# llGuy/madrona_renderer

Hardware: AMD Instinct MI355X
Metric: rendered views/sec (whole node), N worlds x 64x64 RGB+depth (higher is better)
Workload: dtype f32

## Files before the change

include/mrx.h:

```cpp
#ifndef MRX_H
#define MRX_H

#include <stddef.h>
#include <stdint.h>

#ifdef __cplusplus
extern "C" {
#endif

#define MRX_ABI_VERSION 4

enum {
    MRX_OK = 0,
    MRX_E_INVALID = -1,
    MRX_E_NO_DEVICE = -2,
    MRX_E_HIP = -3,
    MRX_E_ASSET = -4,
    MRX_E_UNSUPPORTED = -5
};

enum { MRX_MODE_RASTERIZER = 0, MRX_MODE_RAYTRACER = 1 };

typedef struct {
    float position[3];
// ... 89 lines not shown
    uint32_t max_instances_per_world;
    const mrx_projection *camera_projections;
    const mrx_light *world_lights;
    const uint8_t *instance_colors;
    uint64_t reserved0;
} mrx_config;
#define MRX_CONFIG_V2_SIZE ((uint32_t)offsetof(mrx_config, device_ids))
#define MRX_CONFIG_V4_SIZE ((uint32_t)offsetof(mrx_config, camera_projections))
#define MRX_CONFIG_V4_PROJ_SIZE ((uint32_t)offsetof(mrx_config, world_lights))
#define MRX_CONFIG_V4_LIGHT_SIZE ((uint32_t)offsetof(mrx_config, instance_colors))

typedef struct mrx_renderer mrx_renderer;

enum {
    MRX_BUF_RGB = 0,
    MRX_BUF_DEPTH = 1,
    MRX_BUF_SEGMASK = 2,
    MRX_BUF_INSTANCE_POSITION = 3,
    MRX_BUF_INSTANCE_ROTATION = 4,
    MRX_BUF_CAMERA_POSITION = 5,
    MRX_BUF_CAMERA_ROTATION = 6,
    MRX_BUF_VISIBILITY = 7,
    MRX_BUF_INSTANCE_SCALE = 8,
    MRX_BUF_INSTANCE_OBJECT = 9,
    MRX_BUF_INSTANCE_COLOR = 10,
    MRX_NUM_BUFFERS = 11,
    MRX_BUF_INSTANCE_MATERIAL = 11,
    MRX_NUM_BUFFERS_EXT = 12,
    MRX_BUF_NORMAL = 12,
    MRX_NUM_BUFFERS_EXT2 = 13,
    MRX_BUF_INSTANCE_LABEL = 13,
    MRX_NUM_BUFFERS_EXT3 = 14
};

enum { MRX_DTYPE_U8 = 0, MRX_DTYPE_I32 = 1, MRX_DTYPE_F32 = 2 };

typedef struct {
    uint32_t num_worlds, num_views, num_instances;
    uint32_t num_objects, num_triangles, num_materials, num_textures;
    uint32_t max_world_triangles;
    uint32_t storage_fast, storage_slow;
    int32_t device_id;
    int32_t kernel_variant;
    uint64_t bytes_per_step;
    int32_t render_path;
    uint32_t bvh_nodes;
    uint32_t bvh_depth;
    uint32_t max_world_instances;
    uint32_t num_shards;
} mrx_info_t;
#define MRX_INFO_V2_SIZE ((size_t)offsetof(mrx_info_t, num_shards))

int mrx_create(const mrx_config *cfg, mrx_renderer **out);
void mrx_destroy(mrx_renderer *r);

int mrx_step(mrx_renderer *r);
int mrx_render(mrx_renderer *r);
int mrx_sync(mrx_renderer *r);

void *mrx_buffer(mrx_renderer *r, int which, int64_t dims[4], int *ndim,
                 int *dtype, int *device);

int mrx_supersample(mrx_renderer *r);
void *mrx_sample_buffer(mrx_renderer *r, int which, int64_t dims[4], int *ndim,
                        int *dtype, int *device);
int mrx_resolve(mrx_renderer *r);

int mrx_copy_to_host(mrx_renderer *r, int which, void *dst, uint64_t bytes);

int mrx_refresh_objects(mrx_renderer *r);

int mrx_num_shards(mrx_renderer *r);
mrx_renderer *mrx_shard(mrx_renderer *r, int shard);
void *mrx_buffer_shard(mrx_renderer *r, int shard, int which, int64_t dims[4], int *ndim,
                       int *dtype, int *device);
int64_t mrx_shard_first_world(mrx_renderer *r, int shard);
int64_t mrx_shard_split(uint32_t num_worlds, uint32_t shard, uint32_t num_shards);

enum {
    MRX_ENTRY_NONE = 0, MRX_ENTRY_GROUP_FAST = 1, MRX_ENTRY_GROUP = 2, MRX_ENTRY_CHUNKED = 3,
    MRX_ENTRY_BRUTE = 4, MRX_ENTRY_BVH = 5
};
int mrx_raster_entry(mrx_renderer *r);
enum { MRX_BVH_KERNEL_NONE = 0, MRX_BVH_KERNEL_TILE = 1, MRX_BVH_KERNEL_FLAT = 2 };
typedef struct {
    int32_t kernel;
    uint32_t tile_w, tile_h;
    uint32_t classify;
    uint32_t textured;
    uint32_t record_cap;
    uint32_t record_usable;
    uint32_t tex_cap;
    uint32_t big_cap;
    uint32_t pass_inst;
    uint32_t group_views;
    uint32_t mixed;
    uint32_t priority;
    uint32_t group_tiles;
    int32_t small_area;
    uint32_t workgroups;
} mrx_bvh_launch_t;
int mrx_bvh_launch(mrx_renderer *r, mrx_bvh_launch_t *out);
int mrx_info(mrx_renderer *r, mrx_info_t *out);
int mrx_info_sized(mrx_renderer *r, void *out, size_t size);
void *mrx_stream(mrx_renderer *r);
int mrx_set_stream(mrx_renderer *r, void *stream);

int mrx_time_renders(mrx_renderer *r, int steps, float *ms_total);
int mrx_time_steps_host(mrx_renderer *r, int steps, double *us_per_step);
int64_t mrx_debug_stamps(mrx_renderer *r, uint64_t *dst, int64_t capacity);
int mrx_mark(mrx_renderer *r, int which);
int mrx_elapsed_ms(mrx_renderer *r, float *ms);
int mrx_placement(mrx_renderer *r, float *cand_us, int capacity, float *kept_us);

int mrx_copy_triangles(mrx_renderer *r, float *tri_pos ,
                       float *tri_uv , int32_t *tri_mat ,
                       int32_t *obj_first , int32_t *obj_count );

int mrx_load_obj(const char *path, float **tri_pos, float **tri_uv,
                 uint32_t *num_tris);
int mrx_obj_objects(const char *path, uint32_t *first_tri, uint32_t capacity);
int mrx_decode_png(const char *path, uint8_t **rgba, uint32_t *width,
                   uint32_t *height);
int mrx_decode_texture(const char *path, uint8_t **rgba, uint32_t *width,
                       uint32_t *height);
int mrx_decode_bc7(const uint8_t *blocks, uint32_t num_blocks, uint8_t *rgba );
int64_t mrx_describe_obj_materials(const char *path, char *json, uint64_t capacity);
int mrx_blas_check(const float *tri_pos , uint32_t num_tris, uint32_t *num_nodes,
                   uint32_t *depth, uint32_t *num_leaves);
void mrx_free(void *p);
uint32_t mrx_dispatch_min_tris(uint32_t base, uint32_t num_views, int textured, uint32_t width, uint32_t height,
                               uint32_t num_cus);
uint32_t mrx_group_fill(uint32_t num_cus);
int mrx_dispatch_flat(int raytracer, uint32_t num_views, uint32_t width, uint32_t height, uint32_t max_world_triangles,
                      uint32_t max_world_instances, uint32_t num_cus);

int mrx_set_view_projection(mrx_renderer *r, uint32_t first_view, uint32_t count, const mrx_projection *proj);
int mrx_view_projection(mrx_renderer *r, uint32_t first_view, uint32_t count, mrx_projection *out);
int mrx_projection_constants(uint32_t width, uint32_t height, int render_mode, mrx_projection proj, float out[6]);

int mrx_set_world_light(mrx_renderer *r, uint32_t first_world, uint32_t count, const mrx_light *lights);
int mrx_world_light(mrx_renderer *r, uint32_t first_world, uint32_t count, mrx_light *out);
int mrx_light_constants(mrx_light light, float out[5]);

int mrx_set_instance_materials(mrx_renderer *r, uint32_t first_row, uint32_t count, const int32_t *materials);
int mrx_instance_materials(mrx_renderer *r, uint32_t first_row, uint32_t count, int32_t *out);

int mrx_set_instance_labels(mrx_renderer *r, uint32_t first_row, uint32_t count, const int32_t *labels);
int mrx_instance_labels(mrx_renderer *r, uint32_t first_row, uint32_t count, int32_t *out);

int mrx_device_count(void);
int mrx_abi_version(void);
const char *mrx_last_error(void);

#ifdef __cplusplus
}
#endif
#endif
```

madrona_renderer_amd/build.py:

```python
import os
import shutil
import subprocess
import sys
import sysconfig

HERE = os.path.dirname(os.path.abspath(__file__))
ROOT = os.path.dirname(HERE)
CSRC = os.path.join(HERE, "csrc")
ARCH = "gfx950"

HIP_SOURCES = ["raster.hip", "bvh.hip", "resolve.hip", "bvh.cpp", "mrx_api.cpp", "assets.cpp", "ktx2.cpp"]
HIP_DEPS = HIP_SOURCES + ["raster.hpp", "raster_dev.hpp", "bvh.hpp", "resolve.hpp", "assets.hpp", "bc7_tables.inc",
                          "../../include/mrx.h"]
MGR_SOURCES = ["manager.cpp"]
MGR_DEPS = MGR_SOURCES + ["../../include/madrona_mi355/manager.hpp",
                          "../../include/madrona_mi355/types.hpp", "../../include/mrx.h"]
PY_SOURCES = ["py_module.cpp", "manager.cpp"]


def ext_suffix():
    return sysconfig.get_config_var("EXT_SUFFIX") or ".so"


def lib_path():
    return os.path.join(HERE, "libmrx_hip.so")


def mgr_path():
    return os.path.join(HERE, "libmadrona_mi355.so")


def module_path():
    return os.path.join(HERE, "madrona_renderer" + ext_suffix())


def _stale(target, deps):
    if not os.path.exists(target):
        return True
    t = os.path.getmtime(target)
    return any(os.path.getmtime(os.path.join(CSRC, d)) > t for d in deps)


def _run(cmd, verbose):
    if verbose:
        print("+", " ".join(cmd), flush=True)
    subprocess.check_call(cmd)


def hipcc():
    exe = shutil.which("hipcc") or "/opt/rocm/bin/hipcc"
    if not os.path.exists(exe):
        raise RuntimeError("hipcc not found: the HIP library cannot be built")
    return exe


def build_hip(force=False, verbose=False, extra_flags=()):
    out = lib_path()
    if force or _stale(out, HIP_DEPS):
        cmd = [hipcc(), "--offload-arch=" + ARCH, "-O3", "-std=c++17", "-fPIC",
               "-shared", "-ffp-contract=off", "-fno-fast-math",
               "-mllvm", "-disable-promote-alloca-to-vector",
               "-fno-slp-vectorize",
               "-mllvm", "-amdgpu-kernarg-preload-count=12",
               "-Wall", "-Wno-unused-function"]
        cmd += list(extra_flags)
        cmd += os.environ.get("MRX_EXTRA_HIPCC_FLAGS", "").split()
        cmd += [os.path.join(CSRC, s) for s in HIP_SOURCES]
        cmd += ["-lz", "-ldl", "-Wl,-rpath,/opt/rocm/lib", "-o", out]
        _run(cmd, verbose)
    return out


def build_manager(force=False, verbose=False):
    out = mgr_path()
    if force or _stale(out, MGR_DEPS) or \
            os.path.getmtime(out) < os.path.getmtime(lib_path()):
        cmd = ["g++", "-O2", "-std=c++17", "-fPIC", "-shared", "-Wall"]
        cmd += [os.path.join(CSRC, s) for s in MGR_SOURCES]
        cmd += ["-L" + HERE, "-lmrx_hip", "-Wl,-rpath,$ORIGIN", "-o", out]
        _run(cmd, verbose)
    return out


def build_module(force=False, verbose=False):
    import pybind11
    out = module_path()
    if force or _stale(out, PY_SOURCES + MGR_DEPS) or \
            os.path.getmtime(out) < os.path.getmtime(lib_path()):
        cmd = ["g++", "-O2", "-std=c++17", "-fPIC", "-shared", "-Wall",
               "-fvisibility=hidden",
               "-I" + pybind11.get_include(),
               "-I" + sysconfig.get_paths()["include"]]
        cmd += [os.path.join(CSRC, s) for s in PY_SOURCES]
        cmd += ["-L" + HERE, "-lmrx_hip", "-Wl,-rpath,$ORIGIN", "-o", out]
        _run(cmd, verbose)
# ... 53 lines not shown
```

madrona_renderer_amd/csrc/mrx_api.cpp:

```cpp
#include "../../include/mrx.h"

#include <cmath>
#include <cstdio>
#include <cstdlib>
#include <cstring>
#include <algorithm>
#include <array>
#include <atomic>
#include <chrono>
#include <climits>
#include <map>
#include <string>
#include <thread>
#include <utility>
#include <vector>

#include <linux/futex.h>
#include <sys/syscall.h>
#include <unistd.h>

#include <hip/hip_runtime_api.h>

#include "assets.hpp"
#include "bvh.hpp"
// ... 220 lines not shown
        }
        return e;
    }
    const size_t tb = (px * 4 + kOutPeriod - 1) / kOutPeriod * kOutPeriod;
    const size_t depthOff = wantRgb ? tb + depthPhase : 0;
    const size_t idsOff = wantDepth ? depthOff + tb + kOutPeriod - (depthOff % kOutPeriod) + idsPhase
                                    : wantRgb ? tb + idsPhase : 0;
    const size_t end = (wantIds ? idsOff : wantDepth ? depthOff : 0) + px * 4;
    const size_t normalOff = (end + kOutPeriod - 1) / kOutPeriod * kOutPeriod + normalPhase;
    const size_t total = wantNormal ? normalOff + px * 4 : end;
    const char *how = std::getenv("MRX_OUT_ALLOC");
    int dev = 0;
    (void)hipGetDevice(&dev);
    auto own = [&](auto &buf) {
        return (how && how[0] == 'v') ? buf.allocVmm(px, total - px * 4, dev) : buf.alloc(px, total - px * 4);
    };
    const hipError_t e = wantRgb ? own(rgb) : wantDepth ? own(depth) : own(ids);
    if (e != hipSuccess)
        return e;
    char *base = static_cast<char *>(wantRgb ? rgb.base : wantDepth ? depth.base : ids.base);
    if (wantRgb && wantDepth)
        depth.view(base + depthOff, px);
    if (wantIds && (wantRgb || wantDepth))
        ids.view(base + idsOff, px);
    if (wantNormal)
        normal.view(base + normalOff, px);
    return hipSuccess;
}

}

struct ShardWorker;
static void stopShardWorkers(mrx_renderer *r);

struct mrx_renderer {
    int device = 0;
    hipStream_t stream = nullptr;
    int32_t mode = MRX_MODE_RASTERIZER;
    uint32_t flags = 0;
    int32_t variant = 0;
    uint64_t stepCount = 0;
    mrx_info_t info {};
    mrx::RasterParams params {};
    std::vector<mrx::ObjTri> hostTris;
    std::vector<int32_t> objFirst, objCount;
    DevBuf<mrx::ObjTri> tris;
    DevBuf<mrx::TriMat> triMats;
    DevBuf<mrx::TexDesc> textures;
    DevBuf<uint32_t> texels;
    DevBuf<mrx::WorldTri> viewTris;
    DevBuf<uint32_t> viewTriCount;
    DevBuf<uint8_t> poseBlock, geomBlock;
    DevBuf<float> instPos, instRot, instScale, camPos, camRot;
    DevBuf<int32_t> instObj;
    DevBuf<uint32_t> instColor;
    DevBuf<int32_t> instMat;
    DevBuf<mrx::MatRec> matTable;
    bool anyMatTextured = false;
    int32_t *matStage = nullptr;
    hipEvent_t matEv = nullptr;
    bool matCopyPending = false;
    DevBuf<int32_t> instLabel;
    int32_t *labelStage = nullptr;
    hipEvent_t labelEv = nullptr;
    bool labelCopyPending = false;
    DevBuf<uint32_t> rgb;
    DevBuf<float> depth;
    DevBuf<int32_t> ids;
    DevBuf<uint32_t> normal;
    uint32_t ss = 1;
    DevBuf<uint32_t> outRgb;
    DevBuf<float> outDepth;
    DevBuf<int32_t> outIds;
    DevBuf<uint32_t> outNormal;
    DevBuf<unsigned long long> stamps;
    uint32_t *xccHost = nullptr, *xccDev = nullptr;
    int32_t xcdPhaseForced = -1;
    uint32_t launches = 0;
    DevBuf<mrx::BvhNode> bvhNodes;
    DevBuf<uint32_t> bvhLeafTris, worldInstStart, viewWorld, instKBase;
    DevBuf<mrx::ObjInfo> objInfo;
    bool useBvh = false;
    int32_t lastEntry = mrx::kEntryNone;
    std::vector<int32_t> boundObj;
    std::vector<uint32_t> worldInstStartHost, viewWorldHost, worldCams;
    std::vector<mrx::TriMat> triMatsHost;
    mrx::BlasSet blas;
    uint32_t bvhMinTris = mrx::kBvhMinTris;
    uint32_t bvhGroupTilesGeneral = 1;
    std::vector<mrx_renderer *> shards;
    std::vector<uint32_t> shardFirstWorld;
    std::vector<ShardWorker *> workers;
    std::vector<mrx_renderer *> ownShards;
    uint32_t workerSeq = 0;
    bool shardAsync = false;
    uint32_t rendersPosted = 0;
    mrx_renderer *parent = nullptr;
    hipEvent_t ev0 = nullptr, ev1 = nullptr;
    std::vector<float> placementUs;
    float placementKeptUs = 0.0f;
    std::vector<mrx_projection> proj;
    DevBuf<mrx::ViewProj> projDev;
    mrx::ViewProj *projStage = nullptr;
    hipEvent_t projEv = nullptr;
    bool projCopyPending = false;
    std::vector<mrx_light> lights;
    DevBuf<mrx::ViewLight> lightDev;
    mrx::ViewLight *lightStage = nullptr;

    hipError_t launch()
    {
        const hipError_t e = launchRender();
        return e == hipSuccess && ss > 1 ? launchResolve() : e;
    }

    hipError_t launchResolve()
    {
        mrx::ResolveParams q {};
        q.rgbIn = params.rgb;
        q.depthIn = reinterpret_cast<const uint32_t *>(params.depth);
        q.idsIn = reinterpret_cast<const uint32_t *>(params.ids);
        q.normalIn = params.normal;
        q.rgbOut = outRgb.ptr;
        q.depthOut = reinterpret_cast<uint32_t *>(outDepth.ptr);
        q.idsOut = reinterpret_cast<uint32_t *>(outIds.ptr);
        q.normalOut = outNormal.ptr;
        q.rows = params.numViews * info.storage_slow;
        q.nfast = info.storage_fast;
        q.numCUs = params.numCUs;
        return mrx::launchResolve(q, (int)ss, stream);
    }

    hipError_t launchRender()
    {
        if (xcdPhaseForced >= 0)
            params.xcdPhase = (uint32_t)xcdPhaseForced;
        else if (xccHost)
            params.xcdPhase = *(volatile uint32_t *)xccHost & 1u;
        ++launches;
        params.xccReport = (xccDev && (launches <= 4 || (launches & 31u) == 0)) ? xccDev : nullptr;
        if (useBvh) {
            lastEntry = mrx::kEntryBvh;
            return mrx::launchBvh(params, stream);
        }
        return mrx::launchRaster(params, info.max_world_triangles, variant, stream, &lastEntry);
    }

    ~mrx_renderer()
    {
        stopShardWorkers(this);
        for (mrx_renderer *sh : shards)
            delete sh;
        if (!shards.empty())
            return;
        (void)hipSetDevice(device);
        tris.release(); triMats.release(); textures.release(); texels.release();
        viewTris.release(); viewTriCount.release();
        instPos.release(); instRot.release(); instScale.release();
        camPos.release(); camRot.release(); instObj.release(); instColor.release(); instMat.release();
        instLabel.release();
        matTable.release();
        projDev.release();
        lightDev.release();
        if (projStage)
            (void)hipHostFree(projStage);
        if (lightStage)
            (void)hipHostFree(lightStage);
        if (projEv)
            (void)hipEventDestroy(projEv);
        if (matStage)
            (void)hipHostFree(matStage);
        if (matEv)
            (void)hipEventDestroy(matEv);
        if (labelStage)
            (void)hipHostFree(labelStage);
        if (labelEv)
            (void)hipEventDestroy(labelEv);
        poseBlock.release(); geomBlock.release();
        rgb.release(); depth.release(); ids.release(); normal.release(); stamps.release();
        outRgb.release(); outDepth.release(); outIds.release(); outNormal.release();
        if (xccHost) (void)hipHostFree(xccHost);
        bvhNodes.release(); bvhLeafTris.release(); worldInstStart.release();
        viewWorld.release(); instKBase.release(); objInfo.release();
        if (ev0) (void)hipEventDestroy(ev0);
        if (ev1) (void)hipEventDestroy(ev1);
    }
};


enum : int { kCmdNone = 0, kCmdRender, kCmdSync, kCmdTimed, kCmdResolve, kCmdExit };

struct ShardWorker {
    std::vector<mrx_renderer *> shards;
    std::thread th;
    alignas(64) std::atomic<uint32_t> posted { 0 };
    std::atomic<int> cmd { kCmdNone };
    std::atomic<int> steps { 0 };
    alignas(64) std::atomic<uint32_t> sleeping { 0 };
    alignas(64) std::atomic<uint32_t> done { 0 };
    int rc = MRX_OK;
    std::string err;
    int64_t tSeen = 0, tDone = 0;
    alignas(64) std::atomic<uint32_t> masterSleeping { 0 };
    bool async = false;
    alignas(64) std::atomic<uint32_t> renderPosted { 0 };
    alignas(64) std::atomic<uint32_t> renderDone { 0 };
};

namespace {

inline void cpuRelax() { __builtin_ia32_pause(); }

inline long futexWait(std::atomic<uint32_t> *word, uint32_t expected)
{
    return syscall(SYS_futex, reinterpret_cast<uint32_t *>(word), FUTEX_WAIT_PRIVATE, expected, nullptr, nullptr, 0);
}

inline long futexWake(std::atomic<uint32_t> *word)
{
    return syscall(SYS_futex, reinterpret_cast<uint32_t *>(word), FUTEX_WAKE_PRIVATE, INT_MAX, nullptr, nullptr, 0);
}

int64_t shardSpinNs()
{
    static const int64_t ns = [] {
        const char *e = std::getenv("MRX_SHARD_SPIN_US");
        return (int64_t)(e ? std::max(0, std::atoi(e)) : 200) * 1000;
    }();
    return ns;
}

bool shardTrace()
{
    static const bool on = std::getenv("MRX_SHARD_TRACE") != nullptr;
    return on;
}

struct ShardTrace { int64_t wake = 0, launch = 0, own = 0, total = 0, n = 0; };
thread_local ShardTrace g_trace;

int64_t nowNs()
{
    return std::chrono::duration_cast<std::chrono::nanoseconds>(
               std::chrono::steady_clock::now().time_since_epoch()).count();
}

int groupRun(const std::vector<mrx_renderer *> &shards, int cmd, int steps, bool bindDevice)
{
    if (shards.empty())
        return MRX_OK;
    if (bindDevice)
        MRX_HIP(hipSetDevice(shards[0]->device));
    switch (cmd) {
    case kCmdRender:
        for (mrx_renderer *sh : shards)
            MRX_HIP(sh->launch());
        return MRX_OK;
    case kCmdResolve:
        for (mrx_renderer *sh : shards)
            MRX_HIP(sh->launchResolve());
        return MRX_OK;
    case kCmdSync:
// ... 914 lines not shown
    p.instPos = r.instPos.ptr;
    p.instRot = r.instRot.ptr;
    p.instScale = r.instScale.ptr;
    p.instObj = r.instObj.ptr;
    p.instColor = (cfg.flags & MRX_FLAG_NO_RGB) ? nullptr : r.instColor.ptr;
    p.instMat = (cfg.flags & MRX_FLAG_NO_RGB) ? nullptr : r.instMat.ptr;
    p.matTable = r.matTable.ptr;
    p.numMaterials = wantMats ? (uint32_t)allMats.size() : 0u;
    p.instLabel = (cfg.flags & MRX_FLAG_VISIBILITY_IDS) ? nullptr : r.instLabel.ptr;
    p.camPos = r.camPos.ptr;
    p.camRot = r.camRot.ptr;
    p.rgb = r.rgb.ptr;
    p.depth = r.depth.ptr;
    p.ids = wantIds ? r.ids.ptr : nullptr;
    p.normal = r.normal.ptr;
    p.numViews = nviews;
    {
        int cus = 0;
        MRX_HIP(hipDeviceGetAttribute(&cus, hipDeviceAttributeMultiprocessorCount, r.device));
        p.numCUs = (uint32_t)std::max(cus, 1);
        if (const char *dbg = std::getenv("MRX_FAKE_CUS"))
            p.numCUs = (uint32_t)std::max(1, std::atoi(dbg));
    }
    p.nfast = nfast;
    p.nslow = nslow;
    p.tilesFast = (nfast + 63) / 64;
    p.tilesSlow = (nslow + 63) / 64;
    for (mrx_projection &q : r.proj) {
        mrx::ViewProj c;
        if (projectionConstants(W, H, rt, q, c, &q) != MRX_OK)
            return MRX_E_INVALID;
    }
    p.invFar = rt ? 1.0f / kRtZFar : 0.0f;
    {
        const int rc = applyViewTables(r);
        if (rc != MRX_OK)
            return rc;
    }
    p.transposed = rt ? 1 : 0;
    p.idsAreSegmask = ((rt || wantLabels) && !(cfg.flags & MRX_FLAG_VISIBILITY_IDS)) ? 1 : 0;
    p.debugSkip = 0;
    if (const char *dbg = std::getenv("MRX_DEBUG_SKIP"))
        p.debugSkip = (uint32_t)std::atoi(dbg);
    p.debugStamps = nullptr;
    if (const char *dbg = std::getenv("MRX_DEBUG_STAMPS"))
        if (std::atoi(dbg) != 0) {
            const size_t n = ((size_t)nviews * p.tilesFast * p.tilesSlow * 4 + 64) * 4 * 8;
            MRX_HIP(r.stamps.alloc(n));
            MRX_HIP(hipMemset(r.stamps.ptr, 0, n * sizeof(unsigned long long)));
            p.debugStamps = r.stamps.ptr;
        }
    p.writeThrough = 1;
    if (const char *dbg = std::getenv("MRX_WRITE_THROUGH"))
        p.writeThrough = std::atoi(dbg) != 0;
    p.grpViews = p.grpChunkTiles = p.grpPerView = 0;
    p.grpViewsWanted = p.grpTilesWanted = 0;
    if (const char *dbg = std::getenv("MRX_GROUP_VIEWS"))
        p.grpViewsWanted = std::atoi(dbg);
    if (const char *dbg = std::getenv("MRX_GROUP_TILES"))
        p.grpTilesWanted = std::atoi(dbg);
    p.xcdRotate = 0;
    p.xcdRotateWanted = -1;
    if (const char *dbg = std::getenv("MRX_XCD_ROTATE"))
        p.xcdRotateWanted = std::atoi(dbg);
    p.xccReport = nullptr;
    p.xcdPhase = 0;
    if (hipHostMalloc((void **)&r.xccHost, 64, hipHostMallocMapped) == hipSuccess &&
        hipHostGetDevicePointer((void **)&r.xccDev, r.xccHost, 0) == hipSuccess) {
        *r.xccHost = 0;
        p.xccReport = r.xccDev;
    } else {
        (void)hipGetLastError();
        r.xccHost = nullptr;
    }
    if (const char *dbg = std::getenv("MRX_XCD_PHASE"))
        r.xcdPhaseForced = std::atoi(dbg) & 1;
    p.xcdSkew = 0;
    p.xcdSkewWanted = -1;
    if (const char *dbg = std::getenv("MRX_XCD_SKEW"))
        p.xcdSkewWanted = std::atoi(dbg);
    p.debugSlots = 0;
    if (const char *dbg = std::getenv("MRX_DEBUG_SLOTS"))
        p.debugSlots = std::atoi(dbg);
    p.bvhNodes = r.bvhNodes.ptr;
    p.bvhLeafTris = r.bvhLeafTris.ptr;
    p.numObjects = (uint32_t)r.objFirst.size();
    p.bvhUniInst = p.bvhUniCams = 0;
    if (cfg.num_worlds > 0) {
        bool uni = true;
        const uint32_t rows0 = worldInstStart[1] - worldInstStart[0];
        for (uint32_t w = 1; uni && w < cfg.num_worlds; ++w)
            uni = worldInstStart[w + 1] - worldInstStart[w] == rows0 &&
                  cfg.worlds[w].num_cameras == cfg.worlds[0].num_cameras;
        if (uni && rows0 > 0 && cfg.worlds[0].num_cameras > 0) {
            p.bvhUniInst = rows0;
            p.bvhUniCams = cfg.worlds[0].num_cameras;
        }
    }
    p.worldInstStart = r.worldInstStart.ptr;
    p.viewWorld = r.viewWorld.ptr;
    p.bvhPassInst = std::min<uint32_t>(128u, std::max<uint32_t>(8u, (maxWorldInst + 7u) / 8u * 8u));
    p.bvhTile = 0;
    if (const char *dbg = std::getenv("MRX_BVH_TILE"))
        p.bvhTile = std::max(0, std::min(2, std::atoi(dbg)));
    p.bvhClassify = blas.nodes.empty() ? 0 : 1;
    if (const char *dbg = std::getenv("MRX_BVH_CLASSIFY"))
        p.bvhClassify = std::atoi(dbg) != 0;
    p.bvhSmallArea = 256;
    if (const char *dbg = std::getenv("MRX_BVH_SMALL_AREA"))
        p.bvhSmallArea = std::max(0, std::min(4096, std::atoi(dbg)));
    if (const char *dbg = std::getenv("MRX_BVH_PASS_INST"))
        p.bvhPassInst = std::min<uint32_t>(512u, std::max<uint32_t>(8u, (uint32_t)std::atoi(dbg) / 8u * 8u));
    p.bvhGroupTiles = 1;
    if (maxWorldInst <= p.bvhPassInst) {
        const uint32_t tw = p.bvhTile == 2 ? 32 : 64, thh = p.bvhTile == 0 ? 64 : 32;
        const uint32_t tpv = ((nfast + tw - 1) / tw) * ((nslow + thh - 1) / thh);
        uint32_t g = 1;
        while (g < 16u && g * 2u <= tpv && (uint64_t)nviews * ((tpv + 2u * g - 1) / (2u * g)) >= 2u * p.numCUs)
            g *= 2;
        p.bvhGroupTiles = std::max(1u, g);
        if (const char *dbg = std::getenv("MRX_BVH_GROUP_TILES"))
            p.bvhGroupTiles = (uint32_t)std::max(1, std::min((int)tpv, std::atoi(dbg)));
    }
    r.bvhGroupTilesGeneral = p.bvhGroupTiles;
    mrx_info_t &inf = r.info;
    inf.num_worlds = cfg.num_worlds;
    inf.num_views = nviews;
    inf.num_instances = (uint32_t)instObj.size();
    inf.num_objects = (uint32_t)r.objFirst.size();
    inf.num_triangles = (uint32_t)tris.size();
    inf.num_materials = (uint32_t)allMats.size();
    inf.num_textures = (uint32_t)texDescs.size();
    inf.storage_fast = nfast;
    inf.storage_slow = nslow;
    inf.device_id = r.device;
    inf.kernel_variant = r.variant;
    inf.bvh_nodes = (uint32_t)blas.nodes.size();
    inf.bvh_depth = blas.maxDepth;
    inf.max_world_instances = maxWorldInst;
    inf.num_shards = 1;
    inf.bytes_per_step = (uint64_t)px * (4u * ((r.rgb.ptr ? 1u : 0u) + (r.depth.ptr ? 1u : 0u) + (r.normal.ptr ? 1u : 0u)) +
                                         (wantIds ? 4u : 0u)) +
                         (44ull + (r.instColor.ptr ? 4ull : 0ull) + (r.instMat.ptr ? 4ull : 0ull) +
                          (r.instLabel.ptr ? 4ull : 0ull)) * inf.num_instances +
                         28ull * nviews;
    return bindGeometry(r);
}

}

extern "C" {

int mrx_abi_version(void) { return MRX_ABI_VERSION; }

const char *mrx_last_error(void) { return g_err.c_str(); }

static std::vector<std::pair<mrx_renderer *, uint32_t>> viewOwners(mrx_renderer *r)
{
    std::vector<std::pair<mrx_renderer *, uint32_t>> out;
    uint32_t base = 0;
    if (r->shards.empty()) {
        out.emplace_back(r, 0u);
        return out;
    }
    for (mrx_renderer *sh : r->shards) {
        out.emplace_back(sh, base);
// ... 592 lines not shown
    }
    top->shardFirstWorld.push_back(cfg->num_worlds);
    startShardWorkers(top);
    *out = top;
    return MRX_OK;
}

void mrx_destroy(mrx_renderer *r)
{
    if (!r)
        return;
    stopShardWorkers(r);
    for (mrx_renderer *sh : r->shards) {
        (void)hipSetDevice(sh->device);
        (void)hipStreamSynchronize(sh->stream);
    }
    if (r->shards.empty()) {
        (void)hipSetDevice(r->device);
        (void)hipStreamSynchronize(r->stream);
    }
    delete r;
}

int mrx_render(mrx_renderer *r)
{
    if (r && r->parent) {
        const int src = settle(r);
        if (src != MRX_OK)
            return src;
    }
    if (!r)
        return fail(MRX_E_INVALID, "null renderer");
    if (!r->shards.empty())
        return shardsRun(r, kCmdRender);
    MRX_HIP(hipSetDevice(r->device));
    MRX_HIP(r->launch());
    return MRX_OK;
}

int mrx_step(mrx_renderer *r)
{
    if (!r)
        return fail(MRX_E_INVALID, "null renderer");
    r->stepCount++;
    return mrx_render(r);
}

int mrx_sync(mrx_renderer *r)
{
    if (r && r->parent) {
        const int src = settle(r);
        if (src != MRX_OK)
            return src;
    }
    if (!r)
        return fail(MRX_E_INVALID, "null renderer");
    if (!r->shards.empty())
        return shardsRun(r, kCmdSync);
    MRX_HIP(hipSetDevice(r->device));
    MRX_HIP(hipStreamSynchronize(r->stream));
    return MRX_OK;
}

void *mrx_stream(mrx_renderer *r) { return r ? (void *)r->stream : nullptr; }

static int wantsShard(const char *what)
{
    return fail(MRX_E_UNSUPPORTED, std::string(what) + ": this renderer spans several devices -- "
                                   "address one shard (mrx_shard / mrx_buffer_shard)");
}

static_assert(mrx::kEntryNone == MRX_ENTRY_NONE && mrx::kEntryGroupFast == MRX_ENTRY_GROUP_FAST &&
                  mrx::kEntryGroup == MRX_ENTRY_GROUP && mrx::kEntryChunked == MRX_ENTRY_CHUNKED &&
                  mrx::kEntryBrute == MRX_ENTRY_BRUTE && mrx::kEntryBvh == MRX_ENTRY_BVH,
              "raster.hpp RasterEntry and mrx.h MRX_ENTRY_* disagree");

int mrx_raster_entry(mrx_renderer *r)
{
    if (!r)
        return fail(MRX_E_INVALID, "null renderer");
    return r->shards.empty() ? r->lastEntry : r->shards[0]->lastEntry;
}

int mrx_bvh_launch(mrx_renderer *r, mrx_bvh_launch_t *out)
{
    if (!r)
        return fail(MRX_E_INVALID, "null renderer");
    if (!out)
        return fail(MRX_E_INVALID, "null output");
    const mrx_renderer &sh = r->shards.empty() ? *r : *r->shards[0];
    const mrx::BvhLaunchShape s = mrx::bvhLaunchShape(sh.params);
    mrx_bvh_launch_t o = {};
    o.kernel = !sh.useBvh ? MRX_BVH_KERNEL_NONE : s.flat ? MRX_BVH_KERNEL_FLAT : MRX_BVH_KERNEL_TILE;
    o.tile_w = s.tileW;
    o.tile_h = s.tileH;
    o.classify = s.classify;
    o.textured = s.textured;
    o.record_cap = s.recordCap;
    o.record_usable = s.recordUsable;
    o.tex_cap = s.texCap;
    o.big_cap = s.bigCap;
    o.pass_inst = s.passInst;
    o.group_views = s.groupViews;
    o.mixed = s.mixed;
    o.priority = s.priority;
    o.group_tiles = s.groupTiles;
    o.small_area = s.smallArea;
    o.workgroups = s.workgroups;
    *out = o;
    return MRX_OK;
}

int mrx_num_shards(mrx_renderer *r) { return !r ? 0 : r->shards.empty() ? 1 : (int)r->shards.size(); }

mrx_renderer *mrx_shard(mrx_renderer *r, int shard)
{
    if (!r || shard < 0 || shard >= mrx_num_shards(r)) {
        fail(MRX_E_INVALID, "no such shard");
        return nullptr;
    }
    return r->shards.empty() ? r : r->shards[shard];
}

void *mrx_buffer_shard(mrx_renderer *r, int shard, int which, int64_t dims[4], int *ndim, int *dtype,
                       int *device)
{
    mrx_renderer *sh = mrx_shard(r, shard);
    return sh ? mrx_buffer(sh, which, dims, ndim, dtype, device) : nullptr;
}

int64_t mrx_shard_split(uint32_t num_worlds, uint32_t shard, uint32_t num_shards)
{
    if (num_shards == 0 || shard > num_shards)
        return fail(MRX_E_INVALID, "bad shard");
    return (int64_t)shardFirstWorld(num_worlds, shard, num_shards);
}

int64_t mrx_shard_first_world(mrx_renderer *r, int shard)
{
    if (!r || shard < 0 || shard > mrx_num_shards(r))
        return fail(MRX_E_INVALID, "no such shard");
    if (r->shards.empty())
        return shard == 0 ? 0 : (int64_t)r->info.num_worlds;
    return (int64_t)r->shardFirstWorld[shard];
}

int mrx_refresh_objects(mrx_renderer *r)
{
    {
        const int src = settle(r);
        if (src != MRX_OK)
            return src;
    }
    if (!r)
        return fail(MRX_E_INVALID, "null renderer");
    for (mrx_renderer *sh : r->shards) {
        const int rc = mrx_refresh_objects(sh);
        if (rc != MRX_OK)
            return rc;
    }
    if (!r->shards.empty())
        return MRX_OK;
    MRX_HIP(hipSetDevice(r->device));
    MRX_HIP(hipStreamSynchronize(r->stream));
    std::vector<int32_t> live(r->boundObj.size());
    if (!live.empty())
// ... 454 lines not shown
        return fail(MRX_E_ASSET, err);
    *width = img.width;
    *height = img.height;
    *rgba = (uint8_t *)std::malloc(img.rgba.size() + 4);
    std::memcpy(*rgba, img.rgba.data(), img.rgba.size());
    return MRX_OK;
}

int mrx_decode_texture(const char *path, uint8_t **rgba, uint32_t *width, uint32_t *height)
{
    if (!path || !rgba || !width || !height)
        return fail(MRX_E_INVALID, "null argument");
    mrx::Image img;
    std::string err;
    if (!mrx::decodeTexture(path, img, err))
        return fail(MRX_E_ASSET, err);
    *width = img.width;
    *height = img.height;
    *rgba = (uint8_t *)std::malloc(img.rgba.size() + 4);
    std::memcpy(*rgba, img.rgba.data(), img.rgba.size());
    return MRX_OK;
}

int mrx_decode_bc7(const uint8_t *blocks, uint32_t num_blocks, uint8_t *rgba)
{
    if ((!blocks || !rgba) && num_blocks)
        return fail(MRX_E_INVALID, "null argument");
    for (uint32_t b = 0; b < num_blocks; ++b)
        mrx::decodeBC7Block(blocks + 16 * (size_t)b, reinterpret_cast<uint8_t (*)[4]>(rgba + 64 * (size_t)b));
    return MRX_OK;
}

int64_t mrx_describe_obj_materials(const char *path, char *json, uint64_t capacity)
{
    if (!path || !json)
        return fail(MRX_E_INVALID, "null argument");
    mrx::TriSoup soup;
    std::string err;
    if (!mrx::loadOBJ(path, soup, err))
        return fail(MRX_E_ASSET, err);
    auto quote = [](const std::string &s) {
        std::string o = "\"";
        for (char c : s) {
            if (c == '"' || c == '\\') o += '\\';
            o += c;
        }
        return o + "\"";
    };
    std::string out = "{\"num_tris\":" + std::to_string(soup.numTris()) + ",\"tri_mtl\":[";
    for (size_t i = 0; i < soup.triMtl.size(); ++i)
        out += (i ? "," : "") + std::to_string(soup.triMtl[i]);
    out += "],\"names\":[";
    for (size_t i = 0; i < soup.mtlNames.size(); ++i)
        out += (i ? "," : "") + quote(soup.mtlNames[i]);
    out += "],\"libs\":[";
    for (size_t i = 0; i < soup.mtlLibs.size(); ++i)
        out += (i ? "," : "") + quote(soup.mtlLibs[i]);
    out += "],\"materials\":[";
    std::vector<mrx::MtlMaterial> lib;
    for (const std::string &ml : soup.mtlLibs) {
        std::string merr;
        (void)mrx::loadMTL(ml, lib, merr);
    }
    for (size_t i = 0; i < lib.size(); ++i) {
        char kd[96];
        std::snprintf(kd, sizeof kd, "[%.9g,%.9g,%.9g]", lib[i].kd[0], lib[i].kd[1], lib[i].kd[2]);
        out += std::string(i ? "," : "") + "{\"name\":" + quote(lib[i].name) + ",\"kd\":" + kd +
               ",\"map_kd\":" + quote(lib[i].mapKd) + "}";
    }
    out += "]}";
    if (out.size() + 1 > capacity)
        return fail(MRX_E_INVALID, "buffer too small");
    std::memcpy(json, out.c_str(), out.size() + 1);
    return (int64_t)out.size();
}

uint32_t mrx_dispatch_min_tris(uint32_t base, uint32_t num_views, int textured, uint32_t width, uint32_t height,
                               uint32_t num_cus)
{
    return mrx::bvhDispatchMinTris(base ? base : mrx::kBvhMinTris, num_views, textured != 0, width, height, num_cus);
}

uint32_t mrx_group_fill(uint32_t num_cus) { return mrx::groupFill(num_cus); }

int mrx_dispatch_flat(int raytracer, uint32_t num_views, uint32_t width, uint32_t height, uint32_t max_world_triangles,
                      uint32_t max_world_instances, uint32_t num_cus)
{
    return mrx::bvhDispatchFlat(raytracer != 0, num_views, width, raytracer ? width : height, max_world_triangles,
                                max_world_instances, num_cus) ? 1 : 0;
}

int mrx_blas_check(const float *tri_pos, uint32_t num_tris, uint32_t *num_nodes, uint32_t *depth,
                   uint32_t *num_leaves)
{
    if ((!tri_pos && num_tris) || !num_nodes || !depth || !num_leaves)
        return fail(MRX_E_INVALID, "null argument");
    using namespace mrx;
    std::vector<ObjTri> tris(num_tris);
    for (uint32_t t = 0; t < num_tris; ++t)
        std::memcpy(tris[t].p, tri_pos + 9 * (size_t)t, 36);
    BlasSet b;
    buildBlas(tris.data(), { 0 }, { (int32_t)num_tris }, b);
    *num_nodes = (uint32_t)b.nodes.size();
    *depth = b.maxDepth;
    *num_leaves = 0;
    const ObjInfo &o = b.objects[0];
    if (o.root < 0)
        return num_tris <= kBvhFlatMax && b.nodes.empty() ? MRX_OK
                                                          : fail(MRX_E_INVALID, "large object without a hierarchy");
    if (1 + 7 * b.maxDepth > kBvhStackCap)
        return fail(MRX_E_INVALID, "hierarchy too deep for the traversal stack");
    std::vector<uint32_t> seen(num_tris, 0);
    struct Item { uint32_t node; float lo[3], hi[3]; };
    std::vector<Item> todo;
    {
        Item root {};
        root.node = (uint32_t)o.root;
        std::memcpy(root.lo, o.bbMin, 12);
        std::memcpy(root.hi, o.bbMax, 12);
        todo.push_back(root);
    }
    while (!todo.empty()) {
        const Item it = todo.back();
        todo.pop_back();
        if (it.node >= b.nodes.size())
            return fail(MRX_E_INVALID, "child index out of range");
        const BvhNode &n = b.nodes[it.node];
        for (uint32_t c = 0; c < kBvhWidth; ++c) {
            const uint32_t ref = n.child[c];
            if (ref == kBvhEmpty)
                continue;
            for (int a = 0; a < 3; ++a)
                if (n.bmin[c][a] < it.lo[a] || n.bmax[c][a] > it.hi[a])
                    return fail(MRX_E_INVALID, "child box sticks out of its parent's");
            if (ref & kBvhLeafBit) {
                const uint32_t cnt = ((ref >> kBvhLeafStartBits) & 15u) + 1u;
                const uint32_t start = ref & ((1u << kBvhLeafStartBits) - 1u);
                if (cnt > kBvhLeafMax || start + cnt > b.leafTris.size())
                    return fail(MRX_E_INVALID, "bad leaf");
                ++*num_leaves;
                for (uint32_t i = 0; i < cnt; ++i) {
                    const uint32_t t = b.leafTris[start + i];
                    if (t >= num_tris || seen[t]++)
                        return fail(MRX_E_INVALID, "triangle missing from or repeated in the leaves");
                    for (int v = 0; v < 3; ++v)
                        for (int a = 0; a < 3; ++a) {
                            const float x = tris[t].p[3 * v + a];
                            if (x < n.bmin[c][a] || x > n.bmax[c][a])
                                return fail(MRX_E_INVALID, "triangle outside its leaf's box");
                        }
                }
            } else {
                Item ch {};
                ch.node = ref;
                std::memcpy(ch.lo, n.bmin[c], 12);
                std::memcpy(ch.hi, n.bmax[c], 12);
                todo.push_back(ch);
            }
        }
    }
    for (uint32_t t = 0; t < num_tris; ++t)
        if (seen[t] != 1)
            return fail(MRX_E_INVALID, "triangle missing from the leaves");
    return MRX_OK;
}

// ... 4 lines not shown
```

madrona_renderer_amd/csrc/py_module.cpp:

```cpp
#include <pybind11/numpy.h>
#include <pybind11/pybind11.h>
#include <pybind11/stl.h>

#include <array>
#include <cmath>
#include <cstdio>
#include <string>
#include <vector>

#include "../../include/madrona_mi355/manager.hpp"
#include "../../include/mrx.h"

namespace py = pybind11;

namespace madRender {
namespace detail { void setThrowOnError(bool v); }
}

namespace {

using namespace madRender;

namespace {
struct PyCamera {
// ... 437 lines not shown
        .def("depth_cuda_ptr", [](py::object self, py::object shard) { return self.cast<Manager &>().depthCudaPtr(shardOf(self, shard)); },
             py::arg("shard") = py::none())
        .def("segmask_cuda_ptr", [](py::object self, py::object shard) { return self.cast<Manager &>().segmaskCudaPtr(shardOf(self, shard)); },
             py::arg("shard") = py::none())
        .def("instance_scale_tensor",
             [](py::object self, py::object shard) {
                 return wrapTensor(self, self.cast<Manager &>().instanceScaleTensor(shardOf(self, shard)));
             },
             py::arg("shard") = py::none())
        .def("refresh_objects", &Manager::refreshObjects)
        .def_property_readonly("num_shards", &Manager::numShards)
        .def("shard_first_world", &Manager::shardFirstWorld, py::arg("shard"))
        .def("instance_position_tensor",
             [](py::object self, py::object shard) {
                 return wrapTensor(self, self.cast<Manager &>().instancePositionTensor(shardOf(self, shard)));
             },
             py::arg("shard") = py::none())
        .def("instance_object_tensor",
             [](py::object self, py::object shard) {
                 return wrapTensor(self, self.cast<Manager &>().instanceObjectTensor(shardOf(self, shard)));
             },
             py::arg("shard") = py::none())
        .def("instance_color_tensor",
             [](py::object self, py::object shard) {
                 return wrapTensor(self, self.cast<Manager &>().instanceColorTensor(shardOf(self, shard)));
             },
             py::arg("shard") = py::none())
        .def("instance_label_tensor",
             [](py::object self, py::object shard) {
                 return wrapTensor(self, self.cast<Manager &>().instanceLabelTensor(shardOf(self, shard)));
             },
             py::arg("shard") = py::none())
        .def("instance_material_tensor",
             [](py::object self, py::object shard) {
                 return wrapTensor(self, self.cast<Manager &>().instanceMaterialTensor(shardOf(self, shard)));
             },
             py::arg("shard") = py::none())
        .def("instance_rotation_tensor",
             [](py::object self, py::object shard) {
                 return wrapTensor(self, self.cast<Manager &>().instanceRotationTensor(shardOf(self, shard)));
             },
             py::arg("shard") = py::none())
        .def("camera_position_tensor",
             [](py::object self, py::object shard) {
                 return wrapTensor(self, self.cast<Manager &>().cameraPositionTensor(shardOf(self, shard)));
             },
             py::arg("shard") = py::none())
        .def("camera_rotation_tensor",
             [](py::object self, py::object shard) {
                 return wrapTensor(self, self.cast<Manager &>().cameraRotationTensor(shardOf(self, shard)));
             },
             py::arg("shard") = py::none())
        .def("time_renders", &Manager::timeRenders, py::arg("steps"))
        .def("time_steps_host", &Manager::timeStepsHost, py::arg("steps"))
        .def("mark", &Manager::mark, py::arg("which"))
        .def("elapsed_ms", &Manager::elapsedMs)
        .def("bytes_per_step", &Manager::bytesPerStep)
        .def("render_path", [](Manager &self) { return std::string(self.renderPath()); })
        .def("raster_entry", [](Manager &self) { return std::string(self.rasterEntry()); })
        .def("bvh_launch",
             [](Manager &self) {
                 mrx_bvh_launch_t s = {};
                 if (mrx_bvh_launch(static_cast<mrx_renderer *>(self.nativeHandle()), &s) != MRX_OK)
                     throw std::runtime_error(mrx_last_error());
                 static const char *const kernels[] = {"none", "tile", "flat"};
                 py::dict d;
                 d["kernel"] = kernels[s.kernel >= 0 && s.kernel <= 2 ? s.kernel : 0];
                 d["tile"] = py::make_tuple(s.tile_w, s.tile_h);
                 d["classify"] = s.classify != 0;
                 d["textured"] = s.textured != 0;
                 d["record_cap"] = s.record_cap;
                 d["record_usable"] = s.record_usable;
                 d["tex_cap"] = s.tex_cap;
                 d["big_cap"] = s.big_cap;
                 d["pass_inst"] = s.pass_inst;
                 d["group_views"] = s.group_views;
                 d["mixed"] = s.mixed != 0;
                 d["priority"] = s.priority;
                 d["group_tiles"] = s.group_tiles;
                 d["small_area"] = s.small_area;
                 d["workgroups"] = s.workgroups;
                 return d;
             })
        .def("placement",
             [](Manager &self) {
                 float us[16] = {}, kept = 0.f;
                 const int n = self.placement(us, 16, &kept);
                 py::list cands;
                 for (int i = 0; i < n && i < 16; ++i)
                     cands.append(us[i]);
                 py::dict d;
                 d["tries"] = n > 0 ? n : 1;
                 d["candidates_us"] = cands;
                 d["kept_us"] = n > 0 ? py::object(py::float_(kept)) : py::object(py::none());
                 return d;
             })
        .def("native_handle", [](Manager &self) { return (uint64_t)self.nativeHandle(); })
        .def("set_camera_projection",
             [](Manager &self, py::object vfov, py::object znear, int64_t first_view) {
                 const int64_t total = (int64_t)self.numViews();
                 if (first_view < 0 || first_view > total)
                     throw py::value_error("first_view out of range");
                 auto asVec = [](py::object o, bool &scalar) {
                     std::vector<float> v;
                     scalar = !py::isinstance<py::sequence>(o) && !py::hasattr(o, "__len__");
                     if (scalar)
                         v.push_back(o.cast<float>());
                     else
                         v = py::array_t<float, py::array::c_style | py::array::forcecast>(o).cast<std::vector<float>>();
                     return v;
                 };
                 bool fs = true, zs = true;
                 std::vector<float> fv = asVec(vfov, fs), zv;
                 if (znear.is_none())
                     zv.push_back(0.0f);
                 else {
                     zv = asVec(znear, zs);
                     for (float z : zv)
                         znearOf(z);
                 }
                 if (!fs && !zs && fv.size() != zv.size())
                     throw py::value_error("vfov and znear differ in length");
                 const int64_t n = !fs ? (int64_t)fv.size() : !zs ? (int64_t)zv.size() : total - first_view;
                 if (first_view + n > total)
                     throw py::value_error("more projections than views from first_view on");
                 std::vector<Manager::CameraProjection> proj((size_t)n);
                 for (int64_t i = 0; i < n; ++i) {
                     proj[(size_t)i].vfovDeg = fs ? fv[0] : fv[(size_t)i];
                     proj[(size_t)i].znear = zs ? zv[0] : zv[(size_t)i];
                     checkProjection(proj[(size_t)i]);
                 }
                 if (!self.setViewProjection((uint32_t)first_view, (uint32_t)n, proj.data()))
                     throw py::value_error(mrx_last_error());
             },
             py::arg("vfov"), py::arg("znear") = py::none(), py::arg("first_view") = 0)
        .def("set_world_light",
             [](Manager &self, py::object direction, py::object ambient, py::object diffuse, int64_t first_world) {
                 const int64_t total = (int64_t)self.numWorlds();
                 if (first_world < 0 || first_world > total)
                     throw py::value_error("first_world out of range");
                 const py::array_t<float, py::array::c_style | py::array::forcecast> dir(direction);
                 const bool one = dir.ndim() == 1;
                 if (!((one && dir.shape(0) == 3) || (dir.ndim() == 2 && dir.shape(1) == 3)))
                     throw py::value_error("direction must be one (x, y, z) or an array of shape [n, 3]");
                 auto asVec = [](py::object o, bool &scalar) {
                     std::vector<float> v;
                     scalar = !py::isinstance<py::sequence>(o) && !py::hasattr(o, "__len__");
                     if (scalar)
                         v.push_back(o.cast<float>());
                     else
                         v = py::array_t<float, py::array::c_style | py::array::forcecast>(o).cast<std::vector<float>>();
                     return v;
                 };
                 bool as = true, ds = true;
                 std::vector<float> av, dv;
                 if (!ambient.is_none())
                     av = asVec(ambient, as);
                 if (!diffuse.is_none())
                     dv = asVec(diffuse, ds);
                 int64_t n = one ? -1 : (int64_t)dir.shape(0);
                 for (const auto &sv : { std::make_pair(as, &av), std::make_pair(ds, &dv) })
                     if (!sv.first) {
                         if (n >= 0 && (int64_t)sv.second->size() != n)
                             throw py::value_error("direction, ambient and diffuse differ in length");
                         n = (int64_t)sv.second->size();
                     }
// ... 98 lines not shown
```

madrona_renderer_amd/csrc/raster.hip:

```cpp
#include <hip/hip_runtime.h>
#include <algorithm>
#include <cstdlib>

#include "raster.hpp"
#include "raster_dev.hpp"

namespace mrx {
namespace {

constexpr int kWavesPerBlock = 4;
constexpr int kBruteThreads = kWave * kWavesPerBlock;
constexpr int kChunkedThreads = kWave * kWavesPerBlock, kChunkedWavesPerSimd = 3;
constexpr int kChunk = 64;
constexpr int kHot = 16;
constexpr int kBandRows = 16;
constexpr int kBlocksPerBand = 16;

struct WaveLds {
    float hot[kChunk][kHot];
    float cold[kChunk][kCold];
};

struct TileCtx {
    uint32_t view, tileX0, tileY0;
    uint32_t triBegin, numTris;
    int lx, ly;
};

template <bool PV>
__device__ __forceinline__ bool tileSetup(const RasterParams &p, uint32_t item, int lane,
                                          TileCtx &t, ViewConst &vc, ViewLight &lt)
{
    const uint32_t tilesPerView = p.tilesFast * p.tilesSlow;
    if (item >= p.numViews * tilesPerView)
        return false;
    t.view = item / tilesPerView;
    const uint32_t tile = item % tilesPerView;
    t.tileX0 = (tile % p.tilesFast) * 64u;
    t.tileY0 = (tile / p.tilesFast) * 64u;
    const float4 q = *reinterpret_cast<const float4 *>(p.camRot + 4 * t.view);
    if (PV)
        lt = viewLightOf(p, true, __builtin_amdgcn_readfirstlane(t.view));
    quatToMat(q.x, q.y, q.z, q.w, vc.Rc);
#pragma unroll
    for (int r = 0; r < 3; ++r) {
        vc.c[r] = p.camPos[3 * t.view + r];
        if (PV)
            vc.lv[r] = dot3(vc.Rc[0][r], vc.Rc[1][r], vc.Rc[2][r], lt.toLight[0], lt.toLight[1], lt.toLight[2]);
        else
            vc.lv[r] = dot3(vc.Rc[0][r], vc.Rc[1][r], vc.Rc[2][r],
                            p.toLight[0], p.toLight[1], p.toLight[2]);
    }
#pragma unroll
    for (int r = 0; r < 3; ++r) {
#pragma unroll
        for (int cc = 0; cc < 3; ++cc)
            vc.Rc[r][cc] = __uint_as_float(
                __builtin_amdgcn_readfirstlane(__float_as_uint(vc.Rc[r][cc])));
        vc.c[r] = __uint_as_float(__builtin_amdgcn_readfirstlane(__float_as_uint(vc.c[r])));
        vc.lv[r] = __uint_as_float(__builtin_amdgcn_readfirstlane(__float_as_uint(vc.lv[r])));
    }
    t.triBegin = t.view * p.viewTriStride;
    t.numTris = p.viewTriCount[t.view];
    t.lx = lane & 7;
    t.ly = lane >> 3;
    return true;
}

struct GroupSetupArgs {
    const ObjTri *tris;
    const TriMat *triMats;
    const float *instPos, *instRot, *instScale;
    float sx, ox, sz, oz, s6bPad, ambient, diffuse;
    int32_t transposed;
};

template <bool LAB = false, typename NRMOUT = NoNormalOut>
__device__ __forceinline__ bool setupTriangleProj(const RasterParams &p, const ViewProj &pr, const ViewLight &lt,
                                                  const ViewConst &vc, WorldTri wt, int32_t kWorld, TriPlanes &out,
                                                  float *shade, float *cold, const NRMOUT nrm = NRMOUT())
{
    const GroupSetupArgs sa = { p.tris, p.triMats, p.instPos, p.instRot, p.instScale,
                                pr.sx, pr.ox, pr.sz, pr.oz, pr.s6bPad, lt.ambient, lt.diffuse, p.transposed };
    InstXform x;
    instanceTransform(sa, vc, wt.inst, x);
// ... 411 lines not shown
            dst[1] = make_float4(c.B0, c.B1, c.B2, c.Dy);
            dst[2] = make_float4(c.C0, c.C1, c.C2, c.Dc);
            dst[3] = make_float4(__uint_as_float(mask), 0.f, 0.f, 0.f);
        }
        __syncthreads();

        const uint32_t left = t.numTris - pass;
        const int subs = left >= (uint32_t)kPass ? kWavesPerBlock : (int)((left + kWave - 1) / kWave);
#pragma unroll
        for (int g = 0; g < 4; ++g) {
            const int strip = 2 * wave + (g >> 1), hf = g & 1;
            const uint32_t fy = t.tileY0 + strip * 8 + t.ly;
            const float py = (float)fy;
            const uint32_t fx0 = t.tileX0 + hf * 32 + 4 * t.lx;
            float px[kRegionBlocks];
#pragma unroll
            for (int b = 0; b < kRegionBlocks; ++b)
                px[b] = (float)(fx0 + b);
            for (int sub = 0; sub < subs; ++sub) {
                const uint32_t mask = __float_as_uint(lds.planes[sub * kWave + lane][12]);
                const uint64_t act = __ballot((mask >> (2 * strip + hf)) & 1u);
                if (!(p.debugSkip & 2u))
                    rasterRegion<true, 0>(lds.planes, act, sub * kWave, px, py, invNear, best[g], bid[g]);
            }
#pragma unroll
            for (int b = 0; b < kRegionBlocks; ++b) {
                if (bid[g][b] >= 0) {
                    resolvePixel<IDS>(p, lds.rec, bid[g][b], best[g][b], px[b], py,
                                      outRgba[g][b], outId[g][b]);
                    if (NRM)
                        outNrm[g][b] = nrmLds[bid[g][b]];
                }
                bid[g][b] = -1;
            }
        }
    }

#pragma unroll
    for (int g = 0; g < 4; ++g) {
        const int strip = 2 * wave + (g >> 1), hf = g & 1;
        const uint32_t fy = t.tileY0 + strip * 8 + t.ly;
        const uint32_t fx0 = t.tileX0 + hf * 32 + 4 * t.lx;
        if (NRM)
            outputRegion<IDS, true>(p, t, fx0, fy, invFar, best[g], outRgba[g], outId[g], outNrm[g]);
        else
            outputRegion<IDS>(p, t, fx0, fy, invFar, best[g], outRgba[g], outId[g]);
    }
}

template <bool IDS>
__global__ __launch_bounds__(kChunkedThreads, kChunkedWavesPerSimd)
void rasterChunkedKernel(const RasterParams p)
{
    chunkedKernelBody<IDS, false>(p);
}

template <KernelForm F, bool IDS>
__global__ __launch_bounds__(kChunkedThreads, kChunkedWavesPerSimd)
void rasterChunkedFormKernel(const RasterParams p)
{
    static_assert(F == KernelForm::PV || F == KernelForm::N || F == KernelForm::NPV, "the forms of this family");
    chunkedKernelBody<IDS, formFlags(F).pv, formFlags(F).nrm>(p);
}

constexpr int kGroupTilesMax = 16;
constexpr int kGroupSlotsMax = 256;
constexpr int groupTilesMax(int slots) { return slots <= 128 ? kGroupTilesMax : 8; }

template <int SLOTS, bool PV = false>
struct GroupLds {
    static constexpr int kRecs = SLOTS <= kChunk ? kChunk + 16 : SLOTS;
    static constexpr int kBackground = kRecs;
    float planes[kRecs][16];
    uint32_t live[kRecs];
    float shade[kRecs + 1][4];
    float cold[kRecs][kCold];
    uint32_t masks[groupTilesMax(SLOTS) * (SLOTS <= kChunk ? kChunk : SLOTS)];
    uint32_t tileInfo[kGroupTilesMax][4];
    float tileNear[PV ? kGroupTilesMax : 1];
    uint32_t nextItem;
    uint8_t itemOrder[kGroupTilesMax * 8];
    uint2 items[SLOTS == 16 ? kGroupTilesMax * 8 : 1];
    uint8_t itemPos[SLOTS == 16 ? kGroupTilesMax * 8 : 1];
};
constexpr uint32_t kTileValid = 4u;
constexpr uint32_t kItemValid = 1u << 8;
constexpr uint32_t kItemNearFree = 1u << 9;
constexpr uint32_t kItemAnyTex = 1u << 10;


template <bool IDS, bool FULL, bool TEX, int OUT, bool NRM = false, typename LDS>
__device__ __forceinline__ void storeRegion(const RasterParams &p, const LDS &L, bool doRgb, bool doDepth,
                                            uint32_t *rgbTile, float *depthTile, int32_t *idsTile,
                                            uint32_t pixOff, uint32_t fx0, uint32_t fy,
                                            bool anyTex, const float (&px)[kRegionBlocks], float py,
                                            const float (&best)[kRegionBlocks],
                                            const int32_t (&bid)[kRegionBlocks],
                                            const uint32_t *nrmTab = nullptr, uint32_t *nrmTile = nullptr)
{
    uint32_t nrm[kRegionBlocks];
    if (NRM) {
#pragma unroll
        for (int b = 0; b < kRegionBlocks; ++b)
            nrm[b] = *reinterpret_cast<const uint32_t *>(reinterpret_cast<const char *>(nrmTab) + (bid[b] >> 2));
    }
    uint32_t rgba[kRegionBlocks];
    int32_t id[kRegionBlocks];
    float dep[kRegionBlocks];
    const char *shadeBase = reinterpret_cast<const char *>(&L.shade[0][0]);
#pragma unroll
    for (int b = 0; b < kRegionBlocks; ++b) {
        const float *h = reinterpret_cast<const float *>(shadeBase + bid[b]);
        if (OUT != kOutDepth)
            rgba[b] = __float_as_uint(h[0]);
        if (IDS)
            id[b] = __float_as_int(p.idsAreSegmask ? h[2] : h[3]);
        if (OUT != kOutRGB)
            dep[b] = bid[b] != LDS::kBackground * 16 ? __builtin_amdgcn_rcpf(best[b]) : 0.0f;
    }
    if (TEX && OUT != kOutDepth && anyTex && (OUT != kOutByPointer || doRgb)) {
#pragma unroll
        for (int b = 0; b < kRegionBlocks; ++b) {
            const int32_t rec = bid[b] >> 4;
            const int32_t tex = __float_as_int(L.shade[rec][1]);
            if (tex >= 0)
                rgba[b] = shadeTextured(p, L.cold[rec], tex, px[b], py, 1.0f / best[b]);
        }
    }
    if (p.debugSkip & 1u)
        return;
    if (FULL) {
        if (doRgb)
            streamStore16(p.writeThrough, rgbTile + pixOff, rgba[0], rgba[1], rgba[2], rgba[3]);
        if (doDepth)
            streamStore16(p.writeThrough, depthTile + pixOff, __float_as_uint(dep[0]), __float_as_uint(dep[1]),
                          __float_as_uint(dep[2]), __float_as_uint(dep[3]));
        if (IDS)
            streamStore16(p.writeThrough, idsTile + pixOff, (uint32_t)id[0], (uint32_t)id[1], (uint32_t)id[2], (uint32_t)id[3]);
        if (NRM)
            streamStore16(p.writeThrough, nrmTile + pixOff, nrm[0], nrm[1], nrm[2], nrm[3]);
    } else if (fy < p.nslow) {
#pragma unroll
        for (int b = 0; b < kRegionBlocks; ++b) {
            if (fx0 + b < p.nfast) {
                if (doRgb)
                    streamStore4(p.writeThrough, rgbTile + pixOff + b, rgba[b]);
                if (doDepth)
                    streamStore4(p.writeThrough, depthTile + pixOff + b, __float_as_uint(dep[b]));
                if (IDS)
                    streamStore4(p.writeThrough, idsTile + pixOff + b, (uint32_t)id[b]);
                if (NRM)
                    streamStore4(p.writeThrough, nrmTile + pixOff + b, nrm[b]);
            }
        }
    }
}

template <bool IDS, bool FULL, bool NRM = false>
__device__ __forceinline__ void storeBackground(const RasterParams &p, bool doRgb, bool doDepth, uint32_t *rgbTile,
                                                float *depthTile, int32_t *idsTile,
                                                uint32_t pixOff, uint32_t fx0, uint32_t fy, uint32_t *nrmTile = nullptr)
{
    if (p.debugSkip & 1u)
        return;
    const uint32_t bg = 0xFF000000u;
    if (FULL) {
        if (doRgb)
            streamStore16(p.writeThrough, rgbTile + pixOff, bg, bg, bg, bg);
        if (doDepth)
            streamStore16(p.writeThrough, depthTile + pixOff, 0u, 0u, 0u, 0u);
        if (IDS)
            streamStore16(p.writeThrough, idsTile + pixOff, ~0u, ~0u, ~0u, ~0u);
        if (NRM)
            streamStore16(p.writeThrough, nrmTile + pixOff, kNormalBackground, kNormalBackground, kNormalBackground,
                          kNormalBackground);
    } else if (fy < p.nslow) {
#pragma unroll
        for (int b = 0; b < kRegionBlocks; ++b) {
            if (fx0 + b < p.nfast) {
                if (doRgb)
                    streamStore4(p.writeThrough, rgbTile + pixOff + b, bg);
                if (doDepth)
                    streamStore4(p.writeThrough, depthTile + pixOff + b, 0u);
                if (IDS)
                    streamStore4(p.writeThrough, idsTile + pixOff + b, ~0u);
                if (NRM)
                    streamStore4(p.writeThrough, nrmTile + pixOff + b, kNormalBackground);
            }
        }
    }
}

template <typename LDS>
__device__ __forceinline__ uint32_t classifyPair(const LDS &L, int j, int k, int wave, float invNear, float invFar,
                                                 bool &nearOk, bool &tex)
{
    nearOk = false;
    tex = false;
    const uint32_t info = L.tileInfo[j][3];
    const int rec = (int)(info >> 8) + k;
    if (!(info & kTileValid) || !L.live[rec])
        return 0u;
    const float4 *src = reinterpret_cast<const float4 *>(L.planes[rec]);
    const float4 a = src[0], b = src[1], cc = src[2], bb = src[3];
    TriPlanes c;
    c.A0 = a.x; c.A1 = a.y; c.A2 = a.z; c.Dx = a.w;
    c.B0 = b.x; c.B1 = b.y; c.B2 = b.z; c.Dy = b.w;
    c.C0 = cc.x; c.C1 = cc.y; c.C2 = cc.z; c.Dc = cc.w;
    c.bbX0 = bb.x; c.bbX1 = bb.y; c.bbY0 = bb.z; c.bbY1 = bb.w;
    const uint32_t tx0 = L.tileInfo[j][1], ty0 = L.tileInfo[j][2];
    uint32_t m;
    switch (wave & 3) {
    case 0: m = classifyStrips<0, 2>(c, tx0, ty0, invNear, invFar, nearOk); break;
    case 1: m = classifyStrips<2, 4>(c, tx0, ty0, invNear, invFar, nearOk); break;
    case 2: m = classifyStrips<4, 6>(c, tx0, ty0, invNear, invFar, nearOk); break;
    default: m = classifyStrips<6, 8>(c, tx0, ty0, invNear, invFar, nearOk); break;
    }
    tex = __float_as_int(L.shade[rec][1]) >= 0;
    return m;
}

constexpr int groupWaves(bool tex) { return tex ? 4 : 8; }

template <bool IDS, int SLOTS, bool TEX, int XMODE, bool FAST, int OUT, bool PV = false, bool LT = false, bool COL = false,
          bool MAT = false, bool NRM = false, bool LAB = false>
__device__ __forceinline__ void groupKernelBody(const char *hPose, const char *hGeom, uint32_t hViews, uint32_t hInstances,
                                                uint32_t hPool, uint32_t hShape, uint32_t hGroups, uint32_t hPrefix,
                                                uint32_t hFirst01, uint32_t hFirst23, const RasterParams p)
{
    __shared__ GroupLds<SLOTS, PV> lds;
    constexpr int kBackground = GroupLds<SLOTS, PV>::kBackground;
    __shared__ uint32_t nrmLds[NRM ? GroupLds<SLOTS, PV>::kRecs + 1 : 1];
    const int wave = __builtin_amdgcn_readfirstlane(threadIdx.x / kWave);
    const int lane = threadIdx.x % kWave;
    if (!FAST || wave >= 2)
        touchKernelArguments<(FAST ? 48 : 0) + sizeof(RasterParams)>();
    const uint32_t aNumViews = FAST ? hViews : p.numViews;
    const uint32_t aGrpViews = FAST ? (hShape & 255u) : p.grpViews;
    const uint32_t aXcdSkew = FAST ? ((hShape >> 8) & 15u) : p.xcdSkew;
    const uint32_t aXcdRotate = FAST ? ((hShape >> 12) & 1u) : p.xcdRotate;
    const uint32_t aGrpPerView = FAST ? 1u : p.grpPerView;
    const uint32_t aGrid = FAST ? hGroups : gridDim.x;
    const uint32_t aUniInstances = FAST ? ((hShape >> 13) & 7u) : p.uniInstances;
    const uint32_t aUniCams = FAST ? ((hShape >> 16) & 255u) : p.uniCamsPerWorld;
    const uint32_t dskip = FAST ? 0u : p.debugSkip;
    const PoseLayout lay = poseLayout(hViews, hInstances);
    const float *aCamRot = FAST ? reinterpret_cast<const float *>(hPose + lay.camRot) : p.camRot;
    const float *aCamPos = FAST ? reinterpret_cast<const float *>(hPose + lay.camPos) : p.camPos;
    const int32_t *aInstObj = FAST ? reinterpret_cast<const int32_t *>(hPose + lay.instObj) : p.instObj;
    constexpr bool BYPTR = NRM || LAB;
    const uint32_t *aInstColor = BYPTR ? p.instColor
                                 : FAST ? reinterpret_cast<const uint32_t *>(hPose + lay.total)
                                 : MAT ? reinterpret_cast<const uint32_t *>(p.poseBlock + poseColorOffset(p.numViews, p.numInstances))
                                       : p.instColor;
    const int32_t *aInstMat = BYPTR ? p.instMat
                              : FAST ? reinterpret_cast<const int32_t *>(hPose + lay.total + mrxAlign256(hInstances * 4u))
                                     : p.instMat;
    const uint32_t tilesPerView = FAST ? 1u : p.tilesFast * p.tilesSlow;
    constexpr bool readyItems = FAST && !TEX;
    uint32_t firstView, groupViews, firstTile, groupTiles;
    const uint32_t blk = ((BYPTR ? (p.xcdPhase & 1u) != 0u : (XMODE & 1) != 0) && SLOTS == 16 && aXcdSkew && (blockIdx.x ^ 1u) < aGrid)
                             ? blockIdx.x ^ 1u : blockIdx.x;
    if (((XMODE & 2) || (BYPTR && SLOTS == 16)) && blockIdx.x == 0 && threadIdx.x == (groupWaves(TEX) - 1) * kWave && p.xccReport)
        *p.xccReport = __builtin_amdgcn_s_getreg((3 << 11) | 20);
    uint32_t bid = blk;
    if (aXcdRotate && (bid | 7u) < aGrid)
        bid = (bid & ~7u) | ((bid + 2u * (bid >> 3)) & 7u);
    if (aGrpPerView == 1) {
        firstView = bid * aGrpViews;
        groupViews = aGrpViews;
        firstTile = 0;
        groupTiles = groupViews * tilesPerView;
    } else {
        firstView = bid / aGrpPerView;
        groupViews = 1;
        firstTile = (bid - firstView * aGrpPerView) * p.grpChunkTiles;
        groupTiles = min(p.grpChunkTiles, tilesPerView - firstTile);
    }
    uint32_t firstStrip = 0, numStrips = groupTiles * 8;
    if (SLOTS == 16 && aXcdSkew) {
        if (blk & 1u) {
            firstStrip = aXcdSkew;
            numStrips -= aXcdSkew;
        } else {
            groupViews += 1;
            groupTiles += 1;
            numStrips += aXcdSkew;
        }
    }
    const int groupRecs = (int)groupViews * SLOTS;
    const int numPairs = (int)groupTiles * SLOTS;
    const float invNear = p.invNear, invFar = p.invFar;
    if (dskip & 16u)
        return;
    unsigned long long *stamps = (!FAST && p.debugStamps && wave < 4)
        ? p.debugStamps + ((size_t)blockIdx.x * 4 + wave) * 8 : nullptr;
#define MRX_STAMP(i)                                                           \
    do {                                                                       \
        if (stamps && lane == 0)                                               \
            stamps[i] = __builtin_amdgcn_s_memrealtime();                      \
    } while (0)
    MRX_STAMP(0);
    if (!readyItems)
        for (int i = threadIdx.x; i < numPairs; i += groupWaves(TEX) * kWave)
            lds.masks[i] = 0u;

    if (wave == groupWaves(TEX) - 1 && lane < (int)groupTiles) {
        uint32_t vi = (uint32_t)lane, tile = firstTile;
        if (tilesPerView != 1) {
            vi = groupViews == 1 ? 0u : (uint32_t)lane / tilesPerView;
            tile = firstTile + (uint32_t)lane - vi * tilesPerView;
        }
        const uint32_t ty = tilesPerView != 1 ? tile / p.tilesFast : 0u;
        lds.tileInfo[lane][0] = firstView + vi;
        lds.tileInfo[lane][1] = (tile - ty * p.tilesFast) * 64u;
        lds.tileInfo[lane][2] = ty * 64u;
        lds.tileInfo[lane][3] = (firstView + vi < aNumViews ? kTileValid : 0u) | ((vi * SLOTS) << 8);
        if (PV)
            lds.tileNear[lane] = firstView + vi < aNumViews ? viewProjOf(p, true, firstView + vi).invNear : 0.0f;
    }
    if (wave == groupWaves(TEX) - 1) {
        uint32_t base = 0;
        for (uint32_t c0 = 0; c0 < groupTiles * 8u; c0 += kWave) {
            const uint32_t c = c0 + (uint32_t)lane;
            uint32_t strip = c / groupTiles, tile = c - strip * groupTiles;
            if (tilesPerView != 1) {
                tile = c >> 3;
                strip = c & 7u;
            }
            const uint32_t g = tile * 8u + strip;
            const bool ok = strip < 8u && g >= firstStrip && g < firstStrip + numStrips;
            const uint64_t m = __ballot(ok);
            const uint32_t pos = base + __builtin_popcountll(m & ((1ull << lane) - 1ull));
            if (readyItems) {
                if (strip < 8u)
                    lds.itemPos[g] = ok ? (uint8_t)pos : (uint8_t)0xFF;
            } else if (ok) {
                lds.itemOrder[pos] = (uint8_t)g;
            }
            base += (uint32_t)__builtin_popcountll(m);
        }
    }
    if (wave * kWave < groupRecs) {
        const int rec = wave * kWave + lane;
        const int vi = rec / SLOTS, k = rec % SLOTS;
        const bool recOk = rec < groupRecs;
        const bool viewOk = recOk && firstView + vi < aNumViews;
        const uint32_t view = viewOk ? firstView + vi : 0u;
        WorldTri wt;
        uint32_t numTris;
        if (aUniInstances) {
            const uint32_t kk = (uint32_t)k;
            const uint32_t pre1 = FAST ? (hPrefix & 255u) : p.uniPrefix[1], pre2 = FAST ? ((hPrefix >> 8) & 255u) : p.uniPrefix[2];
            const uint32_t pre3 = FAST ? ((hPrefix >> 16) & 255u) : p.uniPrefix[3], pre4 = FAST ? (hPrefix >> 24) : p.uniPrefix[4];
            const uint32_t ft0 = FAST ? (hFirst01 & 0xFFFFu) : p.uniFirstTri[0], ft1 = FAST ? (hFirst01 >> 16) : p.uniFirstTri[1];
            const uint32_t ft2 = FAST ? (hFirst23 & 0xFFFFu) : p.uniFirstTri[2], ft3 = FAST ? (hFirst23 >> 16) : p.uniFirstTri[3];
            const uint32_t li = (kk >= pre1 ? 1u : 0u) + (kk >= pre2 ? 1u : 0u) + (kk >= pre3 ? 1u : 0u);
            const uint32_t pre = li == 0 ? 0u : li == 1 ? pre1 : li == 2 ? pre2 : pre3;
            const uint32_t first = li == 0 ? ft0 : li == 1 ? ft1 : li == 2 ? ft2 : ft3;
            uint32_t world = view;
            if (aUniCams != 1)
                world = view / aUniCams;
            wt.inst = world * aUniInstances + li;
            wt.tri = first + (kk - pre);
            numTris = viewOk ? pre4 : 0u;
            if (kk >= pre4) {
                wt.inst = 0;
                wt.tri = 0;
            }
        } else {
            wt = p.viewTris[view * p.viewTriStride + ((uint32_t)k < p.viewTriStride ? (uint32_t)k : 0u)];
            numTris = viewOk ? p.viewTriCount[view] : 0u;
        }
        ViewConst vc;
        const ViewLight lt = viewLightOf(p, PV && LT, view);
        {
            const float4 q = *reinterpret_cast<const float4 *>(aCamRot + 4 * view);
            quatToMat(q.x, q.y, q.z, q.w, vc.Rc);
#pragma unroll
            for (int r = 0; r < 3; ++r) {
                vc.c[r] = aCamPos[3 * view + r];
                vc.lv[r] = dot3(vc.Rc[0][r], vc.Rc[1][r], vc.Rc[2][r],
                                lt.toLight[0], lt.toLight[1], lt.toLight[2]);
            }
        }
        TriPlanes c;
        c.A0 = c.B0 = c.C0 = c.A1 = c.B1 = c.C1 = 0.0f;
        c.A2 = c.B2 = c.C2 = c.Dx = c.Dy = c.Dc = 0.0f;
        c.bbX0 = c.bbX1 = c.bbY0 = c.bbY1 = 0.0f;
        bool valid = false;
        MRX_STAMP(1);
        if (recOk) {
            lds.shade[rec][1] = __int_as_float(-1);
            if ((uint32_t)k < numTris && !(dskip & 8u)) {
                const ViewProj pr = viewProjOf(p, PV, view);
                const GroupSetupArgs sa = {
                    FAST ? reinterpret_cast<const ObjTri *>(hGeom) : p.tris,
                    FAST ? reinterpret_cast<const TriMat *>(hGeom + geomMatsOffset(hPool)) : p.triMats,
                    FAST ? reinterpret_cast<const float *>(hPose + lay.instPos) : p.instPos,
                    FAST ? reinterpret_cast<const float *>(hPose + lay.instRot) : p.instRot,
                    FAST ? reinterpret_cast<const float *>(hPose + lay.instScale) : p.instScale,
                    pr.sx, pr.ox, pr.sz, pr.oz, pr.s6bPad, lt.ambient, lt.diffuse, p.transposed };
                InstXform x;
                instanceTransform(sa, vc, wt.inst, x);
                if (BYPTR) {
                    const MatOverride mo = { aInstMat ? aInstMat[wt.inst] : -1, p.numMaterials, p.matTable };
                    if constexpr (NRM)
                        valid = setupTriangleCore<true, true, true, true>(sa, vc.lv, x, wt.tri, aInstObj[wt.inst], k, c,
                                                                          lds.shade[rec], lds.cold[rec],
                                                                          aInstColor ? aInstColor[wt.inst] : 0u, mo,
                                                                          NormalOut { nrmLds + rec });
                    else
                        valid = setupTriangleCore<true, true, true, true>(sa, vc.lv, x, wt.tri, aInstObj[wt.inst], k, c,
                                                                          lds.shade[rec], lds.cold[rec],
                                                                          aInstColor ? aInstColor[wt.inst] : 0u, mo);
                    if (LAB)
                        applyLabel(lds.shade[rec], p.instLabel, wt.inst);
                } else {
                const MatOverride mo = { MAT ? aInstMat[wt.inst] : -1, p.numMaterials, p.matTable };
                valid = setupTriangleCore<true, OUT != kOutDepth, COL, MAT>(sa, vc.lv, x, wt.tri, aInstObj[wt.inst], k, c,
                                                                            lds.shade[rec], lds.cold[rec],
                                                                            COL ? aInstColor[wt.inst] : 0u, mo);
                }
            }
            MRX_STAMP(2);
            float4 *dst = reinterpret_cast<float4 *>(lds.planes[rec]);
            dst[0] = make_float4(c.A0, c.A1, c.A2, c.Dx);
            dst[1] = make_float4(c.B0, c.B1, c.B2, c.Dy);
            dst[2] = make_float4(c.C0, c.C1, c.C2, c.Dc);
            dst[3] = make_float4(c.bbX0, c.bbX1, c.bbY0, c.bbY1);
            lds.live[rec] = (valid && !(dskip & 4u)) ? 1u : 0u;
        }
        if (rec == 0) {
            lds.nextItem = 0;
            lds.shade[kBackground][0] = __uint_as_float(0xFF000000u);
            lds.shade[kBackground][1] = __int_as_float(-1);
            lds.shade[kBackground][2] = __int_as_float(-1);
            lds.shade[kBackground][3] = __int_as_float(-1);
            if (NRM)
                nrmLds[kBackground] = kNormalBackground;
        }
    }
    __syncthreads();
    MRX_STAMP(3);

    constexpr int kPairStride = (groupWaves(TEX) / 4) * kWave;
    for (int pair = (wave >> 2) * kWave + lane; pair - lane < numPairs; pair += kPairStride) {
        if (readyItems) {
            uint32_t m = 0;
            bool nearOk = false, tex = false;
            if (pair < numPairs)
                m = classifyPair(lds, pair / SLOTS, pair % SLOTS, wave, PV ? lds.tileNear[pair / SLOTS] : invNear, invFar,
                                 nearOk, tex);
            m >>= 4 * (wave & 3);
            const uint64_t l0 = __ballot(m & 1u), r0 = __ballot(m & 2u), l1 = __ballot(m & 4u), r1 = __ballot(m & 8u);
            const uint64_t near0 = __ballot((m & 3u) && !nearOk), near1 = __ballot((m & 12u) && !nearOk);
            const uint64_t tex0 = __ballot((m & 3u) && tex), tex1 = __ballot((m & 12u) && tex);
            if (lane % 16 == 0 && pair < numPairs) {
                const uint32_t j = (uint32_t)pair / 16u;
                const uint32_t valid = firstView + j < aNumViews ? kItemValid : 0u;
                const auto put = [&](uint32_t strip, uint64_t l, uint64_t r, uint64_t nearHit, uint64_t texHit) {
                    const uint32_t pos = lds.itemPos[j * 8u + strip];
                    if (pos == 0xFFu)
                        return;
                    const uint32_t desc = j | strip << 4 | valid |
                                          (((nearHit >> lane) & 0xFFFFu) == 0 ? kItemNearFree : 0u) |
                                          (((texHit >> lane) & 0xFFFFu) != 0 ? kItemAnyTex : 0u);
                    lds.items[pos] = make_uint2((uint32_t)((l >> lane) & 0xFFFFu) | (uint32_t)((r >> lane) & 0xFFFFu) << 16,
                                                desc);
                };
                put(2u * (wave & 3), l0, r0, near0, tex0);
                put(2u * (wave & 3) + 1u, l1, r1, near1, tex1);
            }
            continue;
        }
        if (pair >= numPairs)
            continue;
        bool nearOk, tex;
        uint32_t m = classifyPair(lds, pair / SLOTS, pair % SLOTS, wave, PV ? lds.tileNear[pair / SLOTS] : invNear,
                                  invFar, nearOk, tex);
        if (nearOk)
            m |= 1u << (16 + (wave & 3));
        if (m)
            atomicOr(&lds.masks[pair], m);
    }
    __syncthreads();
    MRX_STAMP(4);

    const int lx = lane & 7, ly = lane >> 3;
    const uint32_t laneOff = (uint32_t)ly * p.nfast + 4u * lx;
    int cachedTile = -1, recBase = 0;
    constexpr int SUBS = (SLOTS + kWave - 1) / kWave;
    constexpr int LANES = SLOTS < kWave ? SLOTS : kWave;
    uint32_t view = 0, tileX0 = 0, tileY0 = 0, mask[SUBS] = {};
    float pxTile[2][kRegionBlocks] = {};
    bool anyTex = false, nearFree = false, full = false;
    uint32_t *rgbTile = nullptr;
    float *depthTile = nullptr;
    int32_t *idsTile = nullptr;
    uint32_t *nrmTile = nullptr;
    const bool doRgb = storesRgb<OUT>(p.rgb), doDepth = storesDepth<OUT>(p.depth);
    uint32_t itemMasks = 0;
    float tileNear = invNear;
    if (readyItems) {
        full = (p.nfast & 3u) == 0 && 64u <= p.nfast && 64u <= p.nslow;
#pragma unroll
        for (int hf = 0; hf < 2; ++hf)
#pragma unroll
            for (int b = 0; b < kRegionBlocks; ++b)
                pxTile[hf][b] = (float)(hf * 32 + 4 * lx + b);
    }
    for (;;) {
        uint32_t item = 0;
        if (lane == 0)
            item = atomicAdd(&lds.nextItem, 1u);
        item = __builtin_amdgcn_readfirstlane(item);
        if (item >= numStrips)
            break;
        int j, strip;
        if (readyItems) {
            const uint2 d = lds.items[item];
            itemMasks = __builtin_amdgcn_readfirstlane(d.x);
            const uint32_t desc = __builtin_amdgcn_readfirstlane(d.y);
            if (!(desc & kItemValid))
                continue;
            j = (int)(desc & 15u);
            strip = (int)((desc >> 4) & 7u);
            nearFree = (desc & kItemNearFree) != 0;
            anyTex = (desc & kItemAnyTex) != 0;
            recBase = j * SLOTS;
            if (PV)
                tileNear = __uint_as_float(__builtin_amdgcn_readfirstlane(__float_as_uint(lds.tileNear[j])));
            const size_t tileBase = (size_t)(firstView + (uint32_t)j) * p.nslow * p.nfast;
            rgbTile = p.rgb + tileBase;
            depthTile = p.depth + tileBase;
            idsTile = IDS ? p.ids + tileBase : nullptr;
            nrmTile = NRM ? p.normal + tileBase : nullptr;
        } else {
            item = __builtin_amdgcn_readfirstlane((uint32_t)lds.itemOrder[item]);
            j = (int)(item >> 3);
            strip = (int)(item & 7u);
            if (j != cachedTile) {
                const uint32_t info = __builtin_amdgcn_readfirstlane(lds.tileInfo[j][3]);
                if (!(info & kTileValid))
                    continue;
                cachedTile = j;
                recBase = (int)(info >> 8);
                view = __builtin_amdgcn_readfirstlane(lds.tileInfo[j][0]);
                tileX0 = __builtin_amdgcn_readfirstlane(lds.tileInfo[j][1]);
                tileY0 = __builtin_amdgcn_readfirstlane(lds.tileInfo[j][2]);
                if (PV)
                    tileNear = __uint_as_float(__builtin_amdgcn_readfirstlane(__float_as_uint(lds.tileNear[j])));
                const size_t tileBase = ((size_t)view * p.nslow + tileY0) * p.nfast + tileX0;
                rgbTile = p.rgb + tileBase;
                depthTile = p.depth + tileBase;
                idsTile = IDS ? p.ids + tileBase : nullptr;
                nrmTile = NRM ? p.normal + tileBase : nullptr;
                full = (p.nfast & 3u) == 0 && tileX0 + 64u <= p.nfast && tileY0 + 64u <= p.nslow;
                anyTex = false;
                nearFree = true;
#pragma unroll
                for (int sub = 0; sub < SUBS; ++sub) {
                    const int slot = sub * kWave + lane;
                    mask[sub] = lane < LANES ? lds.masks[j * SLOTS + slot] : 0u;
                    const int32_t tex = lane < LANES ? __float_as_int(lds.shade[recBase + slot][1]) : -1;
                    anyTex = anyTex || __ballot((mask[sub] & 0xFFFFu) != 0 && tex >= 0) != 0;
                    nearFree = nearFree &&
                               __ballot((mask[sub] & 0xFFFFu) != 0 && ((mask[sub] >> 16) & 0xFu) != 0xFu) == 0;
                }
#pragma unroll
                for (int hf = 0; hf < 2; ++hf)
#pragma unroll
                    for (int b = 0; b < kRegionBlocks; ++b)
                        pxTile[hf][b] = (float)(tileX0 + hf * 32 + 4 * lx + b);
            }
        }
        const uint32_t fy = tileY0 + strip * 8 + ly;
        const float py = (float)fy;
#pragma unroll
        for (int hf = 0; hf < 2; ++hf) {
            const uint32_t fx0 = tileX0 + hf * 32 + 4 * lx;
            const uint32_t pixOff = (uint32_t)(strip * 8) * p.nfast + hf * 32 + laneOff;
            uint64_t act[SUBS];
            bool any = false;
#pragma unroll
            for (int sub = 0; sub < SUBS; ++sub) {
                act[sub] = readyItems ? (uint64_t)((itemMasks >> (16 * hf)) & 0xFFFFu)
                                     : __ballot((mask[sub] >> (2 * strip + hf)) & 1u);
                any = any || act[sub] != 0;
            }
            if (!any) {
                if (full)
                    storeBackground<IDS, true, NRM>(p, doRgb, doDepth, rgbTile, depthTile, idsTile, pixOff, fx0, fy, nrmTile);
                else
                    storeBackground<IDS, false, NRM>(p, doRgb, doDepth, rgbTile, depthTile, idsTile, pixOff, fx0, fy, nrmTile);
                continue;
            }
            const float (&px)[kRegionBlocks] = pxTile[hf];
            float best[kRegionBlocks];
            int32_t bid[kRegionBlocks];
#pragma unroll
            for (int b = 0; b < kRegionBlocks; ++b) {
                best[b] = invFar;
                bid[b] = kBackground * 16;
            }
            if (!(dskip & 2u)) {
#pragma unroll
                for (int sub = 0; sub < SUBS; ++sub) {
                    if (SUBS > 1 && act[sub] == 0)
                        continue;
                    if (nearFree)
                        rasterRegion<false, 4>(lds.planes, act[sub], recBase + sub * kWave, px, py, tileNear, best, bid);
                    else
                        rasterRegion<true, 4>(lds.planes, act[sub], recBase + sub * kWave, px, py, tileNear, best, bid);
                }
            }
            if (full)
                storeRegion<IDS, true, TEX, OUT, NRM>(p, lds, doRgb, doDepth, rgbTile, depthTile, idsTile, pixOff, fx0, fy,
                                                      anyTex, px, py, best, bid, nrmLds, nrmTile);
            else
                storeRegion<IDS, false, TEX, OUT, NRM>(p, lds, doRgb, doDepth, rgbTile, depthTile, idsTile, pixOff, fx0, fy,
                                                       anyTex, px, py, best, bid, nrmLds, nrmTile);
        }
    }
    MRX_STAMP(5);
    MRX_STAMP(6);
    if (stamps && lane == 0)
        stamps[7] = ((unsigned long long)__builtin_amdgcn_s_getreg((31 << 11) | 20) << 32) |
                    (unsigned long long)__builtin_amdgcn_s_getreg((31 << 11) | 4);
#undef MRX_STAMP
}

constexpr int groupThreads(bool tex) { return kWave * groupWaves(tex); }
constexpr int groupWavesPerSimd(KernelForm f, int slots, bool tex)
{
    if (tex)
        return slots > 128 ? 3 : 4;
    if (formFlags(f).lt)
        return 6;
    if (f == KernelForm::N)
        return slots >= 128 ? 6 : 8;
    return slots > 128 ? 6 : 8;
}

template <bool IDS, int SLOTS, bool TEX, int XMODE = 0, int OUT = kOutRGBD>
__global__ __launch_bounds__(groupThreads(TEX), groupWavesPerSimd(KernelForm::Uniform, SLOTS, TEX))
void rasterGroupKernel(const RasterParams p)
{
    groupKernelBody<IDS, SLOTS, TEX, XMODE, false, OUT>(nullptr, nullptr, 0u, 0u, 0u, 0u, 0u, 0u, 0u, 0u, p);
}

template <bool IDS, bool TEX, int XMODE, int OUT>
__global__ __launch_bounds__(groupThreads(TEX), groupWavesPerSimd(KernelForm::Uniform, 16, TEX))
void rasterGroupKernelFast(const char *hPose, const char *hGeom, uint32_t hViews, uint32_t hInstances, uint32_t hPool,
                           uint32_t hShape, uint32_t hGroups, uint32_t hPrefix, uint32_t hFirst01, uint32_t hFirst23,
                           const RasterParams p)
{
    groupKernelBody<IDS, 16, TEX, XMODE, true, OUT>(hPose, hGeom, hViews, hInstances, hPool, hShape, hGroups, hPrefix, hFirst01,
                                               hFirst23, p);
}

template <KernelForm F, bool IDS, int SLOTS, bool TEX>
__global__ __launch_bounds__(groupThreads(TEX), groupWavesPerSimd(F, SLOTS, TEX))
void rasterGroupFormKernel(const RasterParams p)
{
    constexpr FormFlags f = formFlags(F);
    static_assert(F != KernelForm::Uniform && F != KernelForm::PVM && (IDS || !f.lab), "the forms of this family");
    groupKernelBody<IDS, SLOTS, TEX, 0, false, kOutByPointer, f.pv, f.lt, f.col, f.mat, f.nrm, f.lab>(
        nullptr, nullptr, 0u, 0u, 0u, 0u, 0u, 0u, 0u, 0u, p);
}

template <KernelForm F, bool IDS, bool TEX>
__global__ __launch_bounds__(groupThreads(TEX), groupWavesPerSimd(F, 16, TEX))
void rasterGroupFormKernelFast(const char *hPose, const char *hGeom, uint32_t hViews, uint32_t hInstances, uint32_t hPool,
                               uint32_t hShape, uint32_t hGroups, uint32_t hPrefix, uint32_t hFirst01, uint32_t hFirst23,
                               const RasterParams p)
{
    constexpr FormFlags f = formFlags(F);
    static_assert(F != KernelForm::Uniform && F != KernelForm::PVM && (IDS || !f.lab), "the forms of this family");
    groupKernelBody<IDS, 16, TEX, 0, true, kOutByPointer, f.pv, f.lt, f.col, f.mat, f.nrm, f.lab>(
        hPose, hGeom, hViews, hInstances, hPool, hShape, hGroups, hPrefix, hFirst01, hFirst23, p);
}

KernelForm tileForm(const RasterParams &p)
{
    if (p.normal && p.viewProj) return KernelForm::NPV;
    if (p.normal)               return KernelForm::N;
    if (p.viewProj)             return KernelForm::PV;
    return KernelForm::Uniform;
}
KernelForm groupForm(const RasterParams &p)
{
    const bool pv = p.viewProj != nullptr;
    if (p.instLabel && p.ids && pv)       return p.normal ? KernelForm::LN : KernelForm::L;
    if (p.normal && pv && p.tablesVary)   return KernelForm::NPV;
    if (p.normal)                         return KernelForm::N;
    if (p.instMat && pv && p.tablesVary)  return KernelForm::PVLM;
    if (p.instMat)                        return KernelForm::M;
    if (p.instColor && pv && p.tablesVary) return KernelForm::PVLC;
    if (p.instColor)                      return KernelForm::C;
    if (pv && p.lightTable)               return KernelForm::PVL;
    if (pv)                               return KernelForm::PV;
    return KernelForm::Uniform;
}

}

hipError_t launchRaster(const RasterParams &p, uint32_t maxWorldTris,
                        int32_t variant, hipStream_t stream, int32_t *entry)
{
    const uint32_t items = p.numViews * p.tilesFast * p.tilesSlow;
    if (items == 0)
        return hipSuccess;
    const dim3 block(kWave * kWavesPerBlock);
    const bool ids = p.ids != nullptr;
    const bool multi = maxWorldTris > (uint32_t)kChunk;
    const bool large = maxWorldTris > (uint32_t)kGroupSlotsMax;
    if (variant == kVariantBrute) {
        if (entry) *entry = kEntryBrute;
        const dim3 grid((items + kWavesPerBlock - 1) / kWavesPerBlock);
        const KernelForm form = tileForm(p);
        const OutSel out = outSelOf(p.rgb, p.depth);
        const auto byIdsMulti = [&](auto f) {
            withBool(ids, [&](auto IDS) { withBool(multi, [&](auto MULTI) { f(IDS, MULTI); }); });
        };
        if (form != KernelForm::Uniform)
            withValue<KernelForm, KernelForm::NPV, KernelForm::N, KernelForm::PV>(form, [&](auto F) {
                byIdsMulti([&](auto IDS, auto MULTI) {
                    rasterBruteFormKernel<decltype(F)::value, decltype(IDS)::value, decltype(MULTI)::value><<<grid, block, 0, stream>>>(p);
                });
            });
        else
            withValue<int, kOutDepth, kOutRGB, kOutRGBD>(out, [&](auto O) {
                byIdsMulti([&](auto IDS, auto MULTI) {
                    rasterBruteKernel<decltype(IDS)::value, decltype(MULTI)::value, decltype(O)::value><<<grid, block, 0, stream>>>(p);
                });
            });
    } else if (large) {
        if (entry) *entry = kEntryChunked;
        const KernelForm form = tileForm(p);
        withBool(ids, [&](auto IDS) {
            constexpr bool kIds = decltype(IDS)::value;
            if (form != KernelForm::Uniform)
                withValue<KernelForm, KernelForm::PV, KernelForm::N, KernelForm::NPV>(form, [&](auto F) {
                    rasterChunkedFormKernel<decltype(F)::value, kIds><<<dim3(items), block, 0, stream>>>(p);
                });
            else
                rasterChunkedKernel<kIds><<<dim3(items), block, 0, stream>>>(p);
        });
    } else {
        int slots = 16;
        while ((uint32_t)slots < maxWorldTris)
            slots *= 2;
        if (p.debugSlots >= slots && p.debugSlots <= kGroupSlotsMax && (p.debugSlots & (p.debugSlots - 1)) == 0)
            slots = p.debugSlots;
        const uint32_t tpv = p.tilesFast * p.tilesSlow;
        const uint32_t maxTiles = (uint32_t)groupTilesMax(slots);
        const uint32_t kFill = groupFill(p.numCUs);
        RasterParams q = p;
        uint32_t vg = 1, ct = tpv, gpv = 1;
        if (tpv == 1) {
            vg = std::max<uint32_t>(1u, (uint32_t)(kChunk / slots));
            if (p.anyTextured)
                vg = std::min<uint32_t>(vg, 2u);
            while (vg > 1 && (p.numViews + vg - 1) / vg < (vg == 2 ? kFill / 2 : kFill))
                vg /= 2;
        } else if (p.anyTextured) {
            ct = std::max<uint32_t>(1u, std::min<uint32_t>(4u, tpv / 4u));
        } else {
            ct = std::min<uint32_t>(tpv, std::min<uint32_t>(maxTiles, 8u));
        }
        if (tpv != 1)
            while (ct > 1 && (uint64_t)p.numViews * ((tpv + ct - 1) / ct) < kFill)
                ct = (ct + 1) / 2;
        if (p.grpViewsWanted > 0 && tpv * (uint32_t)p.grpViewsWanted <= maxTiles &&
            p.grpViewsWanted * slots <= kChunk) {
            vg = (uint32_t)p.grpViewsWanted;
            ct = tpv;
        }
        if (p.grpTilesWanted > 0 && (uint32_t)p.grpTilesWanted <= maxTiles) {
            vg = 1;
            ct = std::min<uint32_t>((uint32_t)p.grpTilesWanted, tpv);
        }
        gpv = (tpv + ct - 1) / ct;
        q.grpViews = vg;
        q.grpChunkTiles = ct;
        q.grpPerView = gpv;
        const uint32_t numGroups = gpv == 1 ? (p.numViews + vg - 1) / vg : p.numViews * gpv;
        const bool skewable = slots == 16 && tpv == 1 && (vg == 4 || vg == 2);
        q.xcdSkew = (skewable && numGroups >= kFill) ? (vg == 4 ? 3u : 1u) : 0u;
        if (p.xcdSkewWanted >= 0)
            q.xcdSkew = skewable ? (uint32_t)(p.xcdSkewWanted < 8 ? p.xcdSkewWanted : 7) : 0u;
        q.xcdRotate = (tpv == 1 && numGroups >= kFill) ? 1u : 0u;
        if (p.xcdRotateWanted >= 0)
            q.xcdRotate = p.xcdRotateWanted ? 1u : 0u;
        const dim3 grid(numGroups);
        const dim3 gblock(kWave * groupWaves(p.anyTextured != 0));
        GroupHeader h {};
        h.pose = p.poseBlock;
        h.geom = p.geomBlock;
        h.views = p.numViews;
        h.instances = p.numInstances;
        h.poolTris = p.poolTris;
        h.groups = numGroups;
        bool fast = slots == 16 && tpv == 1 && gpv == 1 && p.uniInstances != 0 && p.uniCamsPerWorld < 256 && vg < 256 &&
                    p.poseBlock && p.geomBlock && p.debugSkip == 0 && p.debugStamps == nullptr && p.uniPrefix[4] < 256;
        for (int i = 0; i < 4 && fast; ++i)
            fast = p.uniFirstTri[i] < 65536u;
        if (const char *dbg = std::getenv("MRX_GROUP_FAST"))
            fast = fast && std::atoi(dbg) != 0;
        if (entry) *entry = fast ? kEntryGroupFast : kEntryGroup;
        if (fast) {
            h.shape = vg | (q.xcdSkew << 8) | (q.xcdRotate << 12) | (p.uniInstances << 13) | (p.uniCamsPerWorld << 16) | (1u << 31);
            h.prefix = p.uniPrefix[1] | (p.uniPrefix[2] << 8) | (p.uniPrefix[3] << 16) | (p.uniPrefix[4] << 24);
            h.first01 = p.uniFirstTri[0] | (p.uniFirstTri[1] << 16);
            h.first23 = p.uniFirstTri[2] | (p.uniFirstTri[3] << 16);
        }
        const KernelForm form = groupForm(p);
        const bool tex = p.anyTextured != 0;
        const OutSel out = outSelOf(p.rgb, p.depth);
        const int xmode = slots != 16 ? 0 : ((q.xcdSkew && (p.xcdPhase & 1u)) ? 1 : 0) | (p.xccReport ? 2 : 0);
        const auto byTexIds = [&](auto f) {
            withBool(tex, [&](auto TEX) { withBool(ids, [&](auto IDS) { f(IDS, TEX); }); });
        };
        const auto launchFast = [&](auto kernel) {
            kernel<<<grid, gblock, 0, stream>>>(h.pose, h.geom, h.views, h.instances, h.poolTris, h.shape, h.groups, h.prefix,
                                                h.first01, h.first23, q);
        };
        const auto launchPlain = [&](auto kernel) { kernel<<<grid, gblock, 0, stream>>>(q); };
        withValue<int, 16, 32, 64, 128, 256>(slots, [&](auto S) {
            constexpr int kSlots = decltype(S)::value;
            if (form != KernelForm::Uniform) {
                withValue<KernelForm, KernelForm::PV, KernelForm::PVL, KernelForm::C, KernelForm::PVLC, KernelForm::M,
                          KernelForm::PVLM, KernelForm::N, KernelForm::NPV, KernelForm::L, KernelForm::LN>(form, [&](auto F) {
                    constexpr KernelForm kForm = decltype(F)::value;
                    byTexIds([&](auto IDS, auto TEX) {
                        constexpr bool kIds = decltype(IDS)::value, kTex = decltype(TEX)::value;
                        if constexpr (kIds || !formFlags(kForm).lab) {
                            if constexpr (kSlots == 16) {
                                if (fast)
                                    return launchFast(rasterGroupFormKernelFast<kForm, kIds, kTex>);
                            }
                            launchPlain(rasterGroupFormKernel<kForm, kIds, kSlots, kTex>);
                        }
                    });
                });
                return;
            }
            withValue<int, 0, 1, 2, 3>(xmode, [&](auto X) {
                constexpr int kX = decltype(X)::value;
                if constexpr (kX == 0 || kSlots == 16)
                    withValue<int, kOutDepth, kOutRGB, kOutRGBD>(out, [&](auto O) {
                        constexpr int kO = decltype(O)::value, kOP = kO == kOutRGB ? kOutByPointer : kO;
                        if constexpr (kSlots == 16) {
                            if (fast)
                                return byTexIds([&](auto IDS, auto TEX) {
                                    launchFast(rasterGroupKernelFast<decltype(IDS)::value, decltype(TEX)::value, kX, kO>);
                                });
                        }
                        byTexIds([&](auto IDS, auto TEX) {
                            launchPlain(rasterGroupKernel<decltype(IDS)::value, kSlots, decltype(TEX)::value, kX, kOP>);
                        });
                    });
            });
        });
    }
    return hipGetLastError();
}

}
```

madrona_renderer_amd/csrc/raster.hpp:

```cpp
#pragma once

#include <cstdint>
#include <type_traits>
#include <hip/hip_runtime_api.h>

namespace mrx {

struct BvhNode;
struct ObjInfo;

struct alignas(32) ViewProj {
    float sx, ox, sz, oz;
    float invNear, s6bPad;
    float pad[2];
};
static_assert(sizeof(ViewProj) == 32, "ViewProj is one 32-byte record");

struct alignas(32) ViewLight {
    float toLight[3];
    float ambient, diffuse;
    float pad[3];
};
static_assert(sizeof(ViewLight) == 32, "ViewLight is one 32-byte record");

// ... 25 lines not shown
    int32_t tex;
};
static_assert(sizeof(MatRec) == 16, "MatRec is one 16-byte record");

struct WorldTri {
    uint32_t inst;
    uint32_t tri;
};

struct RasterParams {
    const ObjTri *tris;
    const TriMat *triMats;
    const TexDesc *textures;
    const uint32_t *texels;
    int32_t anyTextured;
    const WorldTri *viewTris;
    const uint32_t *viewTriCount;
    uint32_t viewTriStride;
    uint32_t uniInstances;
    uint32_t uniCamsPerWorld;
    uint32_t uniPrefix[5];
    uint32_t uniFirstTri[4];
    const char *poseBlock;
    const char *geomBlock;
    uint32_t numInstances, poolTris;
    const float *instPos;
    const float *instRot;
    const float *instScale;
    const int32_t *instObj;
    const float *camPos;
    const float *camRot;
    uint32_t *rgb;
    float *depth;
    int32_t *ids;
    uint32_t numViews;
    uint32_t nfast, nslow;
    uint32_t tilesFast, tilesSlow;
    float sx, ox, sz, oz;
    float invNear, invFar;
    float s6bPad;
    float toLight[3];
    float ambient, diffuse;
    int32_t transposed;
    int32_t idsAreSegmask;
    uint32_t debugSkip;
    uint32_t writeThrough;
    uint32_t grpViews, grpChunkTiles, grpPerView;
    int32_t grpViewsWanted, grpTilesWanted;
    uint32_t xcdSkew;
    int32_t xcdSkewWanted;
    uint32_t *xccReport;
    uint32_t xcdPhase;
    uint32_t xcdRotate;
    int32_t xcdRotateWanted;
    int32_t debugSlots;
    unsigned long long *debugStamps;
    const BvhNode *bvhNodes;
    const uint32_t *bvhLeafTris;
    const ObjInfo *instInfo;
    uint32_t numObjects;
    uint32_t bvhUniInst, bvhUniCams;
    const uint32_t *worldInstStart;
    const uint32_t *viewWorld;
    const uint32_t *instKBase;
    uint32_t bvhPassInst;
    int32_t bvhTile;
    int32_t bvhSmallArea;
    int32_t bvhClassify;
    uint32_t bvhGroupTiles;
    uint32_t bvhGroupViews;
    uint32_t bvhFlat;
    uint32_t bvhTexCap;
    uint32_t numCUs;
    const ViewProj *viewProj;
    const ViewLight *viewLight;
    uint32_t lightTable;
    uint32_t tablesVary;
    const uint32_t *instColor;
    const int32_t *instMat;
    const MatRec *matTable;
    uint32_t numMaterials;
    uint32_t *normal;
    const int32_t *instLabel;
};

constexpr int32_t kLabelObject = INT32_MIN;

#if defined(__HIP__) || defined(__HIPCC__)
#define MRX_HD __host__ __device__
#else
#define MRX_HD
#endif
struct PoseLayout {
    uint32_t camRot, camPos, instRot, instPos, instScale, instObj, total;
};
MRX_HD inline uint32_t mrxAlign256(uint32_t x) { return (x + 255u) & ~255u; }
MRX_HD inline PoseLayout poseLayout(uint32_t views, uint32_t instances)
{
    PoseLayout l;
    l.camRot = 0;
    l.camPos = l.camRot + mrxAlign256(views * 16u);
    l.instRot = l.camPos + mrxAlign256(views * 12u);
    l.instPos = l.instRot + mrxAlign256(instances * 16u);
    l.instScale = l.instPos + mrxAlign256(instances * 12u);
    l.instObj = l.instScale + mrxAlign256(instances * 12u);
    l.total = l.instObj + mrxAlign256(instances * 4u);
    return l;
}
MRX_HD inline uint32_t poseColorOffset(uint32_t views, uint32_t instances) { return poseLayout(views, instances).total; }
MRX_HD inline uint32_t poseMaterialOffset(uint32_t views, uint32_t instances)
{
    return poseColorOffset(views, instances) + mrxAlign256(instances * 4u);
}
MRX_HD inline uint32_t poseLabelOffset(uint32_t views, uint32_t instances)
{
    return poseMaterialOffset(views, instances) + mrxAlign256(instances * 4u);
}
MRX_HD inline uint32_t geomMatsOffset(uint32_t poolTris) { return mrxAlign256(poolTris * 64u); }

struct GroupHeader {
    const char *pose;
    const char *geom;
    uint32_t views, instances, poolTris;
    uint32_t shape;
    uint32_t groups;
    uint32_t prefix;
    uint32_t first01, first23;
};

constexpr uint32_t kBvhMinTris = 129;

enum OutSel : int {
    kOutRGBD = 0,
    kOutDepth = 1,
    kOutRGB = 2,
    kOutByPointer = 3
};
inline OutSel outSelOf(const void *rgb, const void *depth)
{
    return !rgb ? kOutDepth : !depth ? kOutRGB : kOutRGBD;
}

enum class KernelForm : int {
    Uniform = 0,
    PV, PVL, C, PVLC, M, PVLM, N, NPV, L, LN,
    PVM,
};
struct FormFlags {
    bool pv;
    bool lt;
    bool col;
    bool mat;
    bool nrm;
    bool lab;
};
constexpr FormFlags formFlags(KernelForm f)
{
    switch (f) {
    case KernelForm::PV:   return FormFlags { true,  false, false, false, false, false };
    case KernelForm::PVL:  return FormFlags { true,  true,  false, false, false, false };
    case KernelForm::C:    return FormFlags { false, false, true,  false, false, false };
    case KernelForm::PVLC: return FormFlags { true,  true,  true,  false, false, false };
    case KernelForm::M:    return FormFlags { false, false, true,  true,  false, false };
    case KernelForm::PVLM: return FormFlags { true,  true,  true,  true,  false, false };
    case KernelForm::N:    return FormFlags { false, false, true,  true,  true,  false };
    case KernelForm::NPV:  return FormFlags { true,  true,  true,  true,  true,  false };
    case KernelForm::L:    return FormFlags { true,  true,  true,  true,  false, true };
    case KernelForm::LN:   return FormFlags { true,  true,  true,  true,  true,  true };
    case KernelForm::PVM:  return FormFlags { true,  false, false, true,  false, false };
    default:               return FormFlags { false, false, false, false, false, false };
    }
}

template <typename F>
inline auto withBool(bool b, F &&f)
{
    return b ? f(std::true_type {}) : f(std::false_type {});
}
template <typename T, T V0, T... Vs, typename F>
inline auto withValue(T v, F &&f)
{
    if constexpr (sizeof...(Vs) == 0)
        return f(std::integral_constant<T, V0> {});
    else
        return v == V0 ? f(std::integral_constant<T, V0> {}) : withValue<T, Vs...>(v, f);
}

enum KernelVariant : int32_t {
    kVariantDefault = 0,
    kVariantBrute = 1,
    kVariantBvh = 2,
    kVariantRaster = 3,
    kNumVariants
};

inline uint32_t groupFill(uint32_t numCUs) { return 4u * (numCUs ? numCUs : 256u); }
inline uint32_t bvhDispatchMinTris(uint32_t base, uint32_t numViews, bool anyTextured, uint32_t nfast, uint32_t nslow,
                                   uint32_t numCUs)
{
    const uint32_t cus = numCUs ? numCUs : 256u;
    if (nfast > 64u || nslow > 64u)
        return base;
    if (2ull * numViews <= 5ull * cus)
        return base < 65u ? base : 65u;
    if (numViews <= 4u * cus && !anyTextured)
        return base < 91u ? base : 91u;
    return base;
}

inline bool bvhDispatchFlat(bool raytracer, uint32_t numViews, uint32_t nfast, uint32_t nslow, uint32_t maxWorldTris,
                            uint32_t maxWorldInstances, uint32_t numCUs)
{
    const uint32_t cus = numCUs ? numCUs : 256u;
    const uint64_t tpv = (uint64_t)((nfast + 63u) / 64u) * ((nslow + 63u) / 64u);
    return raytracer && maxWorldTris >= 1u && maxWorldTris <= 64u && maxWorldInstances <= 64u && tpv >= 16u &&
           (uint64_t)numViews * tpv >= 192ull * cus;
}

enum RasterEntry : int32_t {
    kEntryNone = 0, kEntryGroupFast = 1, kEntryGroup = 2, kEntryChunked = 3, kEntryBrute = 4, kEntryBvh = 5,
};
hipError_t launchRaster(const RasterParams &p, uint32_t maxWorldTris,
                        int32_t variant, hipStream_t stream, int32_t *entry = nullptr);

hipError_t launchBvh(const RasterParams &p, hipStream_t stream);
constexpr uint32_t kBvhMaxWorldTris = 0x1FFFFEu;
size_t bvhLdsBytes(uint32_t passInst, bool textured, bool classify, uint32_t groupViews, uint32_t texCap);

struct BvhLaunchShape {
    int32_t flat;
    uint32_t tileW, tileH, classify, textured, recordCap, recordUsable, texCap, bigCap, passInst;
    uint32_t groupViews, mixed, priority, groupTiles, workgroups;
    int32_t smallArea;
};
BvhLaunchShape bvhLaunchShape(const RasterParams &p);

}
```

madrona_renderer_amd/csrc/raster_dev.hpp:

```cpp
#pragma once

#include <hip/hip_runtime.h>

#include "raster.hpp"

namespace mrx {
namespace {

constexpr int kWave = 64;
constexpr int kCold = 12;
constexpr int kRegionBlocks = 4;

template <int OUT>
__device__ __forceinline__ bool storesRgb(const void *rgb)
{
    return OUT == kOutByPointer ? rgb != nullptr : OUT != kOutDepth;
}
template <int OUT>
__device__ __forceinline__ bool storesDepth(const void *depth)
{
    return OUT == kOutByPointer ? depth != nullptr : OUT != kOutRGB;
}

__device__ __forceinline__ float dot3(float ax, float ay, float az,
// ... 275 lines not shown

__device__ __forceinline__ void uvPlanes(const TriPlanes &c, float rad, const float (&uv)[6], float *cold)
{
    cold[0] = __builtin_fmaf(uv[4], c.A2, __builtin_fmaf(uv[2], c.A1, uv[0] * c.A0)) * rad;
    cold[1] = __builtin_fmaf(uv[4], c.B2, __builtin_fmaf(uv[2], c.B1, uv[0] * c.B0)) * rad;
    cold[2] = __builtin_fmaf(uv[4], c.C2, __builtin_fmaf(uv[2], c.C1, uv[0] * c.C0)) * rad;
    cold[3] = __builtin_fmaf(uv[5], c.A2, __builtin_fmaf(uv[3], c.A1, uv[1] * c.A0)) * rad;
    cold[4] = __builtin_fmaf(uv[5], c.B2, __builtin_fmaf(uv[3], c.B1, uv[1] * c.B0)) * rad;
    cold[5] = __builtin_fmaf(uv[5], c.C2, __builtin_fmaf(uv[3], c.C1, uv[1] * c.C0)) * rad;
}

template <typename NRMOUT = NoNormalOut>
__device__ __forceinline__ bool setupTriangle(const RasterParams &p,
                                              const ViewConst &vc,
                                              WorldTri wt, int32_t kWorld,
                                              TriPlanes &out, float *shade, float *cold, const NRMOUT nrm = NRMOUT())
{
    InstXform x;
    instanceTransform(p, vc, wt.inst, x);
    return setupTriangleCore(p, vc.lv, x, wt.tri, p.instObj[wt.inst], kWorld, out, shade, cold, 0u, NoMatOverride(), nrm);
}

typedef const __attribute__((address_space(4))) ViewProj *ConstViewProj;
template <typename PARAMS>
__device__ __forceinline__ ViewProj viewProjOf(const PARAMS &p, bool perView, uint32_t view)
{
    ViewProj r;
    if (perView) {
        const ConstViewProj t = (ConstViewProj)p.viewProj + view;
        r.sx = t->sx; r.ox = t->ox; r.sz = t->sz; r.oz = t->oz;
        r.invNear = t->invNear; r.s6bPad = t->s6bPad;
    } else {
        r.sx = p.sx; r.ox = p.ox; r.sz = p.sz; r.oz = p.oz;
        r.invNear = p.invNear; r.s6bPad = p.s6bPad;
    }
    r.pad[0] = r.pad[1] = 0.0f;
    return r;
}

typedef const __attribute__((address_space(4))) ViewLight *ConstViewLight;
template <typename PARAMS>
__device__ __forceinline__ ViewLight viewLightOf(const PARAMS &p, bool perView, uint32_t view)
{
    ViewLight r;
    if (perView) {
        const ConstViewLight t = (ConstViewLight)p.viewLight + view;
        r.toLight[0] = t->toLight[0]; r.toLight[1] = t->toLight[1]; r.toLight[2] = t->toLight[2];
        r.ambient = t->ambient; r.diffuse = t->diffuse;
    } else {
        r.toLight[0] = p.toLight[0]; r.toLight[1] = p.toLight[1]; r.toLight[2] = p.toLight[2];
        r.ambient = p.ambient; r.diffuse = p.diffuse;
    }
    r.pad[0] = r.pad[1] = r.pad[2] = 0.0f;
    return r;
}

__device__ __forceinline__ uint32_t shadeTextured(const RasterParams &p,
                                                  const float *cold, int32_t tex,
                                                  float px, float py, float tt)
{
    const float u = __builtin_fmaf(cold[0], px, __builtin_fmaf(cold[1], py, cold[2])) * tt;
    const float v = __builtin_fmaf(cold[3], px, __builtin_fmaf(cold[4], py, cold[5])) * tt;
    const TexDesc td = p.textures[tex];
    const int tw = (int)td.width, th = (int)td.height;
    float uf = u - floorf(u);
    float vf = v - floorf(v);
    vf = 1.0f - vf;
    int tx = (int)(uf * (float)tw);
    int ty = (int)(vf * (float)th);
    tx = tx > tw - 1 ? tw - 1 : tx;
    ty = ty > th - 1 ? th - 1 : ty;
    tx = tx < 0 ? 0 : tx;
    ty = ty < 0 ? 0 : ty;
    const uint32_t texel = p.texels[td.offset + (uint32_t)ty * (uint32_t)tw + (uint32_t)tx];
    const uint32_t r = toU8(((float)(texel & 255u) * (1.0f / 255.0f)) * cold[6]);
    const uint32_t g = toU8(((float)((texel >> 8) & 255u) * (1.0f / 255.0f)) * cold[7]);
    const uint32_t b = toU8(((float)((texel >> 16) & 255u) * (1.0f / 255.0f)) * cold[8]);
    return r | (g << 8) | (b << 16) | 0xFF000000u;
}

template <size_t BYTES = sizeof(RasterParams)>
__device__ __forceinline__ void touchKernelArguments()
{
    static_assert(BYTES > 0x180 && BYTES <= 0x240, "seven to nine lines: adjust the offsets below");
    const __attribute__((address_space(4))) char *ka =
        (const __attribute__((address_space(4))) char *)__builtin_amdgcn_kernarg_segment_ptr();
    uint32_t t0, t1, t2, t3, t4, t5, t6, t7, t8;
    if (BYTES > 0x200)
        asm volatile("s_load_dword %0, %9, 0x0\n\ts_load_dword %1, %9, 0x40\n\ts_load_dword %2, %9, 0x80\n\t"
                     "s_load_dword %3, %9, 0xc0\n\ts_load_dword %4, %9, 0x100\n\ts_load_dword %5, %9, 0x140\n\t"
                     "s_load_dword %6, %9, 0x180\n\ts_load_dword %7, %9, 0x1c0\n\ts_load_dword %8, %9, 0x200\n\t"
                     "s_waitcnt lgkmcnt(0)"
                     : "=&s"(t0), "=&s"(t1), "=&s"(t2), "=&s"(t3), "=&s"(t4), "=&s"(t5), "=&s"(t6), "=&s"(t7), "=&s"(t8)
                     : "s"(ka));
    else if (BYTES > 0x1c0)
        asm volatile("s_load_dword %0, %8, 0x0\n\ts_load_dword %1, %8, 0x40\n\ts_load_dword %2, %8, 0x80\n\t"
                     "s_load_dword %3, %8, 0xc0\n\ts_load_dword %4, %8, 0x100\n\ts_load_dword %5, %8, 0x140\n\t"
                     "s_load_dword %6, %8, 0x180\n\ts_load_dword %7, %8, 0x1c0\n\ts_waitcnt lgkmcnt(0)"
                     : "=&s"(t0), "=&s"(t1), "=&s"(t2), "=&s"(t3), "=&s"(t4), "=&s"(t5), "=&s"(t6), "=&s"(t7) : "s"(ka));
    else
        asm volatile("s_load_dword %0, %7, 0x0\n\ts_load_dword %1, %7, 0x40\n\ts_load_dword %2, %7, 0x80\n\t"
                     "s_load_dword %3, %7, 0xc0\n\ts_load_dword %4, %7, 0x100\n\ts_load_dword %5, %7, 0x140\n\t"
                     "s_load_dword %6, %7, 0x180\n\ts_waitcnt lgkmcnt(0)"
                     : "=&s"(t0), "=&s"(t1), "=&s"(t2), "=&s"(t3), "=&s"(t4), "=&s"(t5), "=&s"(t6) : "s"(ka));
}

__device__ __forceinline__ void waveLdsSync()
{
    __builtin_amdgcn_fence(__ATOMIC_RELEASE, "wavefront");
    __builtin_amdgcn_wave_barrier();
    __builtin_amdgcn_fence(__ATOMIC_ACQUIRE, "wavefront");
}

typedef float f32x2 __attribute__((ext_vector_type(2)));

__device__ __forceinline__ f32x2 fma2(f32x2 a, f32x2 b, f32x2 c)
{
    return __builtin_elementwise_fma(a, b, c);
}

struct PlanePairs {
    f32x2 A01, A2D, B01, B2D, C01, C2D;
};

__device__ __forceinline__ PlanePairs loadPlanes(const float (*planes)[16], int k)
{
    const float4 *src = reinterpret_cast<const float4 *>(planes[k]);
    const float4 a = src[0], b = src[1], c = src[2];
    PlanePairs q;
    q.A01 = f32x2{ a.x, a.y }; q.A2D = f32x2{ a.z, a.w };
    q.B01 = f32x2{ b.x, b.y }; q.B2D = f32x2{ b.z, b.w };
    q.C01 = f32x2{ c.x, c.y }; q.C2D = f32x2{ c.z, c.w };
    return q;
}

typedef uint32_t u32x4 __attribute__((ext_vector_type(4)));
__device__ __forceinline__ void streamStore16(uint32_t writeThrough, void *dst,
                                              uint32_t a, uint32_t b, uint32_t c, uint32_t d)
{
    const u32x4 v = { a, b, c, d };
    if (writeThrough)
        asm volatile("global_store_dwordx4 %0, %1, off sc1\n\ts_nop 1" :: "v"(dst), "v"(v) : "memory");
    else
        asm volatile("global_store_dwordx4 %0, %1, off\n\ts_nop 1" :: "v"(dst), "v"(v) : "memory");
}
__device__ __forceinline__ u32x4 streamLoad16(const void *src)
{
    u32x4 v;
    asm volatile("global_load_dwordx4 %0, %1, off sc1\n\ts_waitcnt vmcnt(0)" : "=&v"(v) : "v"(src) : "memory");
    return v;
}
__device__ __forceinline__ uint32_t streamLoad4(const void *src)
{
    uint32_t v;
    asm volatile("global_load_dword %0, %1, off sc1\n\ts_waitcnt vmcnt(0)" : "=&v"(v) : "v"(src) : "memory");
    return v;
}
__device__ __forceinline__ void streamStore4(uint32_t writeThrough, void *dst, uint32_t a)
{
    if (writeThrough)
        asm volatile("global_store_dword %0, %1, off sc1" :: "v"(dst), "v"(a) : "memory");
    else
        asm volatile("global_store_dword %0, %1, off" :: "v"(dst), "v"(a) : "memory");
}

}
}
```

Before: 187.3 million.

## Add dynamic view pool so resident workgroups pull extra view groups atomically

Moves the group raster phases into a loop in which workgroups, after finishing their statically assigned views, claim more views from a global atomic pool counter. The last finisher resets the counters. The aim is to balance uneven per-view work and reduce tail idle time across CUs. It adds global atomics, a per-group loop around setup, classify and raster phases, and register pressure from variables that are no longer const.

After: 82.58 million. 55.9% lower.

```diff
diff --git a/include/mrx.h b/include/mrx.h
--- a/include/mrx.h
+++ b/include/mrx.h
@@ -195,6 +195,14 @@
     MRX_ENTRY_BRUTE = 4, MRX_ENTRY_BVH = 5
 };
 int mrx_raster_entry(mrx_renderer *r);
+typedef struct mrx_view_pool {
+    int32_t on;
+    uint32_t groups;
+    uint32_t static_views;
+    uint32_t first_view, size;
+    uint32_t words[2];
+} mrx_view_pool_t;
+int mrx_view_pool(mrx_renderer *r, int shard, mrx_view_pool_t *out);
 enum { MRX_BVH_KERNEL_NONE = 0, MRX_BVH_KERNEL_TILE = 1, MRX_BVH_KERNEL_FLAT = 2 };
 typedef struct {
     int32_t kernel;
@@ -245,6 +253,8 @@
 uint32_t mrx_dispatch_min_tris(uint32_t base, uint32_t num_views, int textured, uint32_t width, uint32_t height,
                                uint32_t num_cus);
 uint32_t mrx_group_fill(uint32_t num_cus);
+int mrx_view_pool_split(int shape_ok, uint32_t num_views, uint32_t group_views, uint32_t fill, uint32_t resident, int mode,
+                        int share8, mrx_view_pool_t *out);
 int mrx_dispatch_flat(int raytracer, uint32_t num_views, uint32_t width, uint32_t height, uint32_t max_world_triangles,
                       uint32_t max_world_instances, uint32_t num_cus);
 
diff --git a/madrona_renderer_amd/build.py b/madrona_renderer_amd/build.py
--- a/madrona_renderer_amd/build.py
+++ b/madrona_renderer_amd/build.py
@@ -10,7 +10,7 @@
 ARCH = "gfx950"
 
 HIP_SOURCES = ["raster.hip", "bvh.hip", "resolve.hip", "bvh.cpp", "mrx_api.cpp", "assets.cpp", "ktx2.cpp"]
-HIP_DEPS = HIP_SOURCES + ["raster.hpp", "raster_dev.hpp", "bvh.hpp", "resolve.hpp", "assets.hpp", "bc7_tables.inc",
+HIP_DEPS = HIP_SOURCES + ["raster.hpp", "raster_dev.hpp", "raster_group_phases.inc", "bvh.hpp", "resolve.hpp", "assets.hpp", "bc7_tables.inc",
                           "../../include/mrx.h"]
 MGR_SOURCES = ["manager.cpp"]
 MGR_DEPS = MGR_SOURCES + ["../../include/madrona_mi355/manager.hpp",
diff --git a/madrona_renderer_amd/csrc/mrx_api.cpp b/madrona_renderer_amd/csrc/mrx_api.cpp
--- a/madrona_renderer_amd/csrc/mrx_api.cpp
+++ b/madrona_renderer_amd/csrc/mrx_api.cpp
@@ -326,6 +326,8 @@
     DevBuf<mrx::ObjInfo> objInfo;
     bool useBvh = false;
     int32_t lastEntry = mrx::kEntryNone;
+    DevBuf<uint32_t> viewPool;
+    mrx::ViewPoolSplit lastPool {};
     std::vector<int32_t> boundObj;
     std::vector<uint32_t> worldInstStartHost, viewWorldHost, worldCams;
     std::vector<mrx::TriMat> triMatsHost;
@@ -385,9 +387,10 @@
         params.xccReport = (xccDev && (launches <= 4 || (launches & 31u) == 0)) ? xccDev : nullptr;
         if (useBvh) {
             lastEntry = mrx::kEntryBvh;
+            lastPool = mrx::ViewPoolSplit {};
             return mrx::launchBvh(params, stream);
         }
-        return mrx::launchRaster(params, info.max_world_triangles, variant, stream, &lastEntry);
+        return mrx::launchRaster(params, info.max_world_triangles, variant, stream, &lastEntry, &lastPool);
     }
 
     ~mrx_renderer()
@@ -421,7 +424,7 @@
         if (labelEv)
             (void)hipEventDestroy(labelEv);
         poseBlock.release(); geomBlock.release();
-        rgb.release(); depth.release(); ids.release(); normal.release(); stamps.release();
+        rgb.release(); depth.release(); ids.release(); normal.release(); stamps.release(); viewPool.release();
         outRgb.release(); outDepth.release(); outIds.release(); outNormal.release();
         if (xccHost) (void)hipHostFree(xccHost);
         bvhNodes.release(); bvhLeafTris.release(); worldInstStart.release();
@@ -1502,6 +1505,16 @@
     p.debugSlots = 0;
     if (const char *dbg = std::getenv("MRX_DEBUG_SLOTS"))
         p.debugSlots = std::atoi(dbg);
+    MRX_HIP(r.viewPool.alloc(2));
+    MRX_HIP(hipMemset(r.viewPool.ptr, 0, 2 * sizeof(uint32_t)));
+    p.viewPool = r.viewPool.ptr;
+    p.poolFirstView = 0;
+    p.viewPoolMode = 1;
+    if (const char *dbg = std::getenv("MRX_VIEW_POOL"))
+        p.viewPoolMode = std::atoi(dbg);
+    p.viewPoolShare = 2;
+    if (const char *dbg = std::getenv("MRX_VIEW_POOL_SHARE"))
+        p.viewPoolShare = std::atoi(dbg);
     p.bvhNodes = r.bvhNodes.ptr;
     p.bvhLeafTris = r.bvhLeafTris.ptr;
     p.numObjects = (uint32_t)r.objFirst.size();
@@ -2260,6 +2273,31 @@
     return r->shards.empty() ? r->lastEntry : r->shards[0]->lastEntry;
 }
 
+int mrx_view_pool(mrx_renderer *r, int shard, mrx_view_pool_t *out)
+{
+    if (!r || !out)
+        return fail(MRX_E_INVALID, "null argument");
+    if (!r->shards.empty()) {
+        if (shard < 0 || (size_t)shard >= r->shards.size())
+            return fail(MRX_E_INVALID, "shard out of range");
+        r = r->shards[(size_t)shard];
+    } else if (shard != 0) {
+        return fail(MRX_E_INVALID, "shard out of range");
+    }
+    const mrx::ViewPoolSplit &s = r->lastPool;
+    out->on = (int32_t)s.on;
+    out->groups = s.groups;
+    out->static_views = s.staticViews;
+    out->first_view = s.firstView;
+    out->size = s.size;
+    out->words[0] = out->words[1] = 0;
+    if (r->viewPool.ptr) {
+        MRX_HIP(hipSetDevice(r->device));
+        MRX_HIP(hipMemcpy(out->words, r->viewPool.ptr, sizeof out->words, hipMemcpyDeviceToHost));
+    }
+    return MRX_OK;
+}
+
 int mrx_bvh_launch(mrx_renderer *r, mrx_bvh_launch_t *out)
 {
     if (!r)
@@ -2880,6 +2918,21 @@
 }
 
 uint32_t mrx_group_fill(uint32_t num_cus) { return mrx::groupFill(num_cus); }
+
+int mrx_view_pool_split(int shape_ok, uint32_t num_views, uint32_t group_views, uint32_t fill, uint32_t resident, int mode,
+                        int share8, mrx_view_pool_t *out)
+{
+    if (!out)
+        return fail(MRX_E_INVALID, "null argument");
+    const mrx::ViewPoolSplit s = mrx::viewPoolSplit(shape_ok != 0, num_views, group_views, fill, resident, mode, share8);
+    out->on = (int32_t)s.on;
+    out->groups = s.groups;
+    out->static_views = s.staticViews;
+    out->first_view = s.firstView;
+    out->size = s.size;
+    out->words[0] = out->words[1] = 0;
+    return MRX_OK;
+}
 
 int mrx_dispatch_flat(int raytracer, uint32_t num_views, uint32_t width, uint32_t height, uint32_t max_world_triangles,
                       uint32_t max_world_instances, uint32_t num_cus)
diff --git a/madrona_renderer_amd/csrc/py_module.cpp b/madrona_renderer_amd/csrc/py_module.cpp
--- a/madrona_renderer_amd/csrc/py_module.cpp
+++ b/madrona_renderer_amd/csrc/py_module.cpp
@@ -543,6 +543,21 @@
                  d["workgroups"] = s.workgroups;
                  return d;
              })
+        .def("view_pool",
+             [](Manager &self, int shard) {
+                 mrx_view_pool_t v = {};
+                 if (mrx_view_pool(static_cast<mrx_renderer *>(self.nativeHandle()), shard, &v) != MRX_OK)
+                     throw std::runtime_error(mrx_last_error());
+                 py::dict d;
+                 d["on"] = v.on != 0;
+                 d["groups"] = v.groups;
+                 d["static_views"] = v.static_views;
+                 d["first_view"] = v.first_view;
+                 d["size"] = v.size;
+                 d["words"] = py::make_tuple(v.words[0], v.words[1]);
+                 return d;
+             },
+             py::arg("shard") = 0)
         .def("placement",
              [](Manager &self) {
                  float us[16] = {}, kept = 0.f;
diff --git a/madrona_renderer_amd/csrc/raster.hip b/madrona_renderer_amd/csrc/raster.hip
--- a/madrona_renderer_amd/csrc/raster.hip
+++ b/madrona_renderer_amd/csrc/raster.hip
@@ -1,6 +1,7 @@
 #include <hip/hip_runtime.h>
 #include <algorithm>
 #include <cstdlib>
+#include <type_traits>
 
 #include "raster.hpp"
 #include "raster_dev.hpp"
@@ -578,6 +579,7 @@
     uint8_t itemOrder[kGroupTilesMax * 8];
     uint2 items[SLOTS == 16 ? kGroupTilesMax * 8 : 1];
     uint8_t itemPos[SLOTS == 16 ? kGroupTilesMax * 8 : 1];
+    uint32_t poolNext;
 };
 constexpr uint32_t kTileValid = 4u;
 constexpr uint32_t kItemValid = 1u << 8;
@@ -728,7 +730,7 @@
     constexpr int kBackground = GroupLds<SLOTS, PV>::kBackground;
     __shared__ uint32_t nrmLds[NRM ? GroupLds<SLOTS, PV>::kRecs + 1 : 1];
     const int wave = __builtin_amdgcn_readfirstlane(threadIdx.x / kWave);
-    const int lane = threadIdx.x % kWave;
+    int lane = threadIdx.x % kWave;
     if (!FAST || wave >= 2)
         touchKernelArguments<(FAST ? 48 : 0) + sizeof(RasterParams)>();
     const uint32_t aNumViews = FAST ? hViews : p.numViews;
@@ -784,8 +786,8 @@
             numStrips += aXcdSkew;
         }
     }
-    const int groupRecs = (int)groupViews * SLOTS;
-    const int numPairs = (int)groupTiles * SLOTS;
+    int groupRecs = (int)groupViews * SLOTS;
+    int numPairs = (int)groupTiles * SLOTS;
     const float invNear = p.invNear, invFar = p.invFar;
     if (dskip & 16u)
         return;
@@ -797,334 +799,49 @@
             stamps[i] = __builtin_amdgcn_s_memrealtime();                      \
     } while (0)
     MRX_STAMP(0);
-    if (!readyItems)
-        for (int i = threadIdx.x; i < numPairs; i += groupWaves(TEX) * kWave)
-            lds.masks[i] = 0u;
-
-    if (wave == groupWaves(TEX) - 1 && lane < (int)groupTiles) {
-        uint32_t vi = (uint32_t)lane, tile = firstTile;
-        if (tilesPerView != 1) {
-            vi = groupViews == 1 ? 0u : (uint32_t)lane / tilesPerView;
-            tile = firstTile + (uint32_t)lane - vi * tilesPerView;
-        }
-        const uint32_t ty = tilesPerView != 1 ? tile / p.tilesFast : 0u;
-        lds.tileInfo[lane][0] = firstView + vi;
-        lds.tileInfo[lane][1] = (tile - ty * p.tilesFast) * 64u;
-        lds.tileInfo[lane][2] = ty * 64u;
-        lds.tileInfo[lane][3] = (firstView + vi < aNumViews ? kTileValid : 0u) | ((vi * SLOTS) << 8);
-        if (PV)
-            lds.tileNear[lane] = firstView + vi < aNumViews ? viewProjOf(p, true, firstView + vi).invNear : 0.0f;
-    }
-    if (wave == groupWaves(TEX) - 1) {
-        uint32_t base = 0;
-        for (uint32_t c0 = 0; c0 < groupTiles * 8u; c0 += kWave) {
-            const uint32_t c = c0 + (uint32_t)lane;
-            uint32_t strip = c / groupTiles, tile = c - strip * groupTiles;
-            if (tilesPerView != 1) {
-                tile = c >> 3;
-                strip = c & 7u;
-            }
-            const uint32_t g = tile * 8u + strip;
-            const bool ok = strip < 8u && g >= firstStrip && g < firstStrip + numStrips;
-            const uint64_t m = __ballot(ok);
-            const uint32_t pos = base + __builtin_popcountll(m & ((1ull << lane) - 1ull));
-            if (readyItems) {
-                if (strip < 8u)
-                    lds.itemPos[g] = ok ? (uint8_t)pos : (uint8_t)0xFF;
-            } else if (ok) {
-                lds.itemOrder[pos] = (uint8_t)g;
-            }
-            base += (uint32_t)__builtin_popcountll(m);
-        }
-    }
-    if (wave * kWave < groupRecs) {
-        const int rec = wave * kWave + lane;
-        const int vi = rec / SLOTS, k = rec % SLOTS;
-        const bool recOk = rec < groupRecs;
-        const bool viewOk = recOk && firstView + vi < aNumViews;
-        const uint32_t view = viewOk ? firstView + vi : 0u;
-        WorldTri wt;
-        uint32_t numTris;
-        if (aUniInstances) {
-            const uint32_t kk = (uint32_t)k;
-            const uint32_t pre1 = FAST ? (hPrefix & 255u) : p.uniPrefix[1], pre2 = FAST ? ((hPrefix >> 8) & 255u) : p.uniPrefix[2];
-            const uint32_t pre3 = FAST ? ((hPrefix >> 16) & 255u) : p.uniPrefix[3], pre4 = FAST ? (hPrefix >> 24) : p.uniPrefix[4];
-            const uint32_t ft0 = FAST ? (hFirst01 & 0xFFFFu) : p.uniFirstTri[0], ft1 = FAST ? (hFirst01 >> 16) : p.uniFirstTri[1];
-            const uint32_t ft2 = FAST ? (hFirst23 & 0xFFFFu) : p.uniFirstTri[2], ft3 = FAST ? (hFirst23 >> 16) : p.uniFirstTri[3];
-            const uint32_t li = (kk >= pre1 ? 1u : 0u) + (kk >= pre2 ? 1u : 0u) + (kk >= pre3 ? 1u : 0u);
-            const uint32_t pre = li == 0 ? 0u : li == 1 ? pre1 : li == 2 ? pre2 : pre3;
-            const uint32_t first = li == 0 ? ft0 : li == 1 ? ft1 : li == 2 ? ft2 : ft3;
-            uint32_t world = view;
-            if (aUniCams != 1)
-                world = view / aUniCams;
-            wt.inst = world * aUniInstances + li;
-            wt.tri = first + (kk - pre);
-            numTris = viewOk ? pre4 : 0u;
-            if (kk >= pre4) {
-                wt.inst = 0;
-                wt.tri = 0;
-            }
-        } else {
-            wt = p.viewTris[view * p.viewTriStride + ((uint32_t)k < p.viewTriStride ? (uint32_t)k : 0u)];
-            numTris = viewOk ? p.viewTriCount[view] : 0u;
-        }
-        ViewConst vc;
-        const ViewLight lt = viewLightOf(p, PV && LT, view);
-        {
-            const float4 q = *reinterpret_cast<const float4 *>(aCamRot + 4 * view);
-            quatToMat(q.x, q.y, q.z, q.w, vc.Rc);
-#pragma unroll
-            for (int r = 0; r < 3; ++r) {
-                vc.c[r] = aCamPos[3 * view + r];
-                vc.lv[r] = dot3(vc.Rc[0][r], vc.Rc[1][r], vc.Rc[2][r],
-                                lt.toLight[0], lt.toLight[1], lt.toLight[2]);
-            }
-        }
-        TriPlanes c;
-        c.A0 = c.B0 = c.C0 = c.A1 = c.B1 = c.C1 = 0.0f;
-        c.A2 = c.B2 = c.C2 = c.Dx = c.Dy = c.Dc = 0.0f;
-        c.bbX0 = c.bbX1 = c.bbY0 = c.bbY1 = 0.0f;
-        bool valid = false;
-        MRX_STAMP(1);
-        if (recOk) {
-            lds.shade[rec][1] = __int_as_float(-1);
-            if ((uint32_t)k < numTris && !(dskip & 8u)) {
-                const ViewProj pr = viewProjOf(p, PV, view);
-                const GroupSetupArgs sa = {
-                    FAST ? reinterpret_cast<const ObjTri *>(hGeom) : p.tris,
-                    FAST ? reinterpret_cast<const TriMat *>(hGeom + geomMatsOffset(hPool)) : p.triMats,
-                    FAST ? reinterpret_cast<const float *>(hPose + lay.instPos) : p.instPos,
-                    FAST ? reinterpret_cast<const float *>(hPose + lay.instRot) : p.instRot,
-                    FAST ? reinterpret_cast<const float *>(hPose + lay.instScale) : p.instScale,
-                    pr.sx, pr.ox, pr.sz, pr.oz, pr.s6bPad, lt.ambient, lt.diffuse, p.transposed };
-                InstXform x;
-                instanceTransform(sa, vc, wt.inst, x);
-                if (BYPTR) {
-                    const MatOverride mo = { aInstMat ? aInstMat[wt.inst] : -1, p.numMaterials, p.matTable };
-                    if constexpr (NRM)
-                        valid = setupTriangleCore<true, true, true, true>(sa, vc.lv, x, wt.tri, aInstObj[wt.inst], k, c,
-                                                                          lds.shade[rec], lds.cold[rec],
-                                                                          aInstColor ? aInstColor[wt.inst] : 0u, mo,
-                                                                          NormalOut { nrmLds + rec });
-                    else
-                        valid = setupTriangleCore<true, true, true, true>(sa, vc.lv, x, wt.tri, aInstObj[wt.inst], k, c,
-                                                                          lds.shade[rec], lds.cold[rec],
-                                                                          aInstColor ? aInstColor[wt.inst] : 0u, mo);
-                    if (LAB)
-                        applyLabel(lds.shade[rec], p.instLabel, wt.inst);
-                } else {
-                const MatOverride mo = { MAT ? aInstMat[wt.inst] : -1, p.numMaterials, p.matTable };
-                valid = setupTriangleCore<true, OUT != kOutDepth, COL, MAT>(sa, vc.lv, x, wt.tri, aInstObj[wt.inst], k, c,
-                                                                            lds.shade[rec], lds.cold[rec],
-                                                                            COL ? aInstColor[wt.inst] : 0u, mo);
-                }
-            }
-            MRX_STAMP(2);
-            float4 *dst = reinterpret_cast<float4 *>(lds.planes[rec]);
-            dst[0] = make_float4(c.A0, c.A1, c.A2, c.Dx);
-            dst[1] = make_float4(c.B0, c.B1, c.B2, c.Dy);
-            dst[2] = make_float4(c.C0, c.C1, c.C2, c.Dc);
-            dst[3] = make_float4(c.bbX0, c.bbX1, c.bbY0, c.bbY1);
-            lds.live[rec] = (valid && !(dskip & 4u)) ? 1u : 0u;
-        }
-        if (rec == 0) {
-            lds.nextItem = 0;
-            lds.shade[kBackground][0] = __uint_as_float(0xFF000000u);
-            lds.shade[kBackground][1] = __int_as_float(-1);
-            lds.shade[kBackground][2] = __int_as_float(-1);
-            lds.shade[kBackground][3] = __int_as_float(-1);
-            if (NRM)
-                nrmLds[kBackground] = kNormalBackground;
-        }
-    }
-    __syncthreads();
-    MRX_STAMP(3);
-
-    constexpr int kPairStride = (groupWaves(TEX) / 4) * kWave;
-    for (int pair = (wave >> 2) * kWave + lane; pair - lane < numPairs; pair += kPairStride) {
-        if (readyItems) {
-            uint32_t m = 0;
-            bool nearOk = false, tex = false;
-            if (pair < numPairs)
-                m = classifyPair(lds, pair / SLOTS, pair % SLOTS, wave, PV ? lds.tileNear[pair / SLOTS] : invNear, invFar,
-                                 nearOk, tex);
-            m >>= 4 * (wave & 3);
-            const uint64_t l0 = __ballot(m & 1u), r0 = __ballot(m & 2u), l1 = __ballot(m & 4u), r1 = __ballot(m & 8u);
-            const uint64_t near0 = __ballot((m & 3u) && !nearOk), near1 = __ballot((m & 12u) && !nearOk);
-            const uint64_t tex0 = __ballot((m & 3u) && tex), tex1 = __ballot((m & 12u) && tex);
-            if (lane % 16 == 0 && pair < numPairs) {
-                const uint32_t j = (uint32_t)pair / 16u;
-                const uint32_t valid = firstView + j < aNumViews ? kItemValid : 0u;
-                const auto put = [&](uint32_t strip, uint64_t l, uint64_t r, uint64_t nearHit, uint64_t texHit) {
-                    const uint32_t pos = lds.itemPos[j * 8u + strip];
-                    if (pos == 0xFFu)
-                        return;
-                    const uint32_t desc = j | strip << 4 | valid |
-                                          (((nearHit >> lane) & 0xFFFFu) == 0 ? kItemNearFree : 0u) |
-                                          (((texHit >> lane) & 0xFFFFu) != 0 ? kItemAnyTex : 0u);
-                    lds.items[pos] = make_uint2((uint32_t)((l >> lane) & 0xFFFFu) | (uint32_t)((r >> lane) & 0xFFFFu) << 16,
-                                                desc);
-                };
-                put(2u * (wave & 3), l0, r0, near0, tex0);
-                put(2u * (wave & 3) + 1u, l1, r1, near1, tex1);
-            }
-            continue;
-        }
-        if (pair >= numPairs)
-            continue;
-        bool nearOk, tex;
-        uint32_t m = classifyPair(lds, pair / SLOTS, pair % SLOTS, wave, PV ? lds.tileNear[pair / SLOTS] : invNear,
-                                  invFar, nearOk, tex);
-        if (nearOk)
-            m |= 1u << (16 + (wave & 3));
-        if (m)
-            atomicOr(&lds.masks[pair], m);
-    }
-    __syncthreads();
-    MRX_STAMP(4);
-
-    const int lx = lane & 7, ly = lane >> 3;
-    const uint32_t laneOff = (uint32_t)ly * p.nfast + 4u * lx;
-    int cachedTile = -1, recBase = 0;
-    constexpr int SUBS = (SLOTS + kWave - 1) / kWave;
-    constexpr int LANES = SLOTS < kWave ? SLOTS : kWave;
-    uint32_t view = 0, tileX0 = 0, tileY0 = 0, mask[SUBS] = {};
-    float pxTile[2][kRegionBlocks] = {};
-    bool anyTex = false, nearFree = false, full = false;
-    uint32_t *rgbTile = nullptr;
-    float *depthTile = nullptr;
-    int32_t *idsTile = nullptr;
-    uint32_t *nrmTile = nullptr;
-    const bool doRgb = storesRgb<OUT>(p.rgb), doDepth = storesDepth<OUT>(p.depth);
-    uint32_t itemMasks = 0;
-    float tileNear = invNear;
-    if (readyItems) {
-        full = (p.nfast & 3u) == 0 && 64u <= p.nfast && 64u <= p.nslow;
-#pragma unroll
-        for (int hf = 0; hf < 2; ++hf)
-#pragma unroll
-            for (int b = 0; b < kRegionBlocks; ++b)
-                pxTile[hf][b] = (float)(hf * 32 + 4 * lx + b);
-    }
-    for (;;) {
-        uint32_t item = 0;
-        if (lane == 0)
-            item = atomicAdd(&lds.nextItem, 1u);
-        item = __builtin_amdgcn_readfirstlane(item);
-        if (item >= numStrips)
-            break;
-        int j, strip;
-        if (readyItems) {
-            const uint2 d = lds.items[item];
-            itemMasks = __builtin_amdgcn_readfirstlane(d.x);
-            const uint32_t desc = __builtin_amdgcn_readfirstlane(d.y);
-            if (!(desc & kItemValid))
-                continue;
-            j = (int)(desc & 15u);
-            strip = (int)((desc >> 4) & 7u);
-            nearFree = (desc & kItemNearFree) != 0;
-            anyTex = (desc & kItemAnyTex) != 0;
-            recBase = j * SLOTS;
-            if (PV)
-                tileNear = __uint_as_float(__builtin_amdgcn_readfirstlane(__float_as_uint(lds.tileNear[j])));
-            const size_t tileBase = (size_t)(firstView + (uint32_t)j) * p.nslow * p.nfast;
-            rgbTile = p.rgb + tileBase;
-            depthTile = p.depth + tileBase;
-            idsTile = IDS ? p.ids + tileBase : nullptr;
-            nrmTile = NRM ? p.normal + tileBase : nullptr;
-        } else {
-            item = __builtin_amdgcn_readfirstlane((uint32_t)lds.itemOrder[item]);
-            j = (int)(item >> 3);
-            strip = (int)(item & 7u);
-            if (j != cachedTile) {
-                const uint32_t info = __builtin_amdgcn_readfirstlane(lds.tileInfo[j][3]);
-                if (!(info & kTileValid))
-                    continue;
-                cachedTile = j;
-                recBase = (int)(info >> 8);
-                view = __builtin_amdgcn_readfirstlane(lds.tileInfo[j][0]);
-                tileX0 = __builtin_amdgcn_readfirstlane(lds.tileInfo[j][1]);
-                tileY0 = __builtin_amdgcn_readfirstlane(lds.tileInfo[j][2]);
-                if (PV)
-                    tileNear = __uint_as_float(__builtin_amdgcn_readfirstlane(__float_as_uint(lds.tileNear[j])));
-                const size_t tileBase = ((size_t)view * p.nslow + tileY0) * p.nfast + tileX0;
-                rgbTile = p.rgb + tileBase;
-                depthTile = p.depth + tileBase;
-                idsTile = IDS ? p.ids + tileBase : nullptr;
-                nrmTile = NRM ? p.normal + tileBase : nullptr;
-                full = (p.nfast & 3u) == 0 && tileX0 + 64u <= p.nfast && tileY0 + 64u <= p.nslow;
-                anyTex = false;
-                nearFree = true;
-#pragma unroll
-                for (int sub = 0; sub < SUBS; ++sub) {
-                    const int slot = sub * kWave + lane;
-                    mask[sub] = lane < LANES ? lds.masks[j * SLOTS + slot] : 0u;
-                    const int32_t tex = lane < LANES ? __float_as_int(lds.shade[recBase + slot][1]) : -1;
-                    anyTex = anyTex || __ballot((mask[sub] & 0xFFFFu) != 0 && tex >= 0) != 0;
-                    nearFree = nearFree &&
-                               __ballot((mask[sub] & 0xFFFFu) != 0 && ((mask[sub] >> 16) & 0xFu) != 0xFu) == 0;
-                }
-#pragma unroll
-                for (int hf = 0; hf < 2; ++hf)
-#pragma unroll
-                    for (int b = 0; b < kRegionBlocks; ++b)
-                        pxTile[hf][b] = (float)(tileX0 + hf * 32 + 4 * lx + b);
-            }
-        }
-        const uint32_t fy = tileY0 + strip * 8 + ly;
-        const float py = (float)fy;
-#pragma unroll
-        for (int hf = 0; hf < 2; ++hf) {
-            const uint32_t fx0 = tileX0 + hf * 32 + 4 * lx;
-            const uint32_t pixOff = (uint32_t)(strip * 8) * p.nfast + hf * 32 + laneOff;
-            uint64_t act[SUBS];
-            bool any = false;
-#pragma unroll
-            for (int sub = 0; sub < SUBS; ++sub) {
-                act[sub] = readyItems ? (uint64_t)((itemMasks >> (16 * hf)) & 0xFFFFu)
-                                     : __ballot((mask[sub] >> (2 * strip + hf)) & 1u);
-                any = any || act[sub] != 0;
-            }
-            if (!any) {
-                if (full)
-                    storeBackground<IDS, true, NRM>(p, doRgb, doDepth, rgbTile, depthTile, idsTile, pixOff, fx0, fy, nrmTile);
-                else
-                    storeBackground<IDS, false, NRM>(p, doRgb, doDepth, rgbTile, depthTile, idsTile, pixOff, fx0, fy, nrmTile);
-                continue;
-            }
-            const float (&px)[kRegionBlocks] = pxTile[hf];
-            float best[kRegionBlocks];
-            int32_t bid[kRegionBlocks];
-#pragma unroll
-            for (int b = 0; b < kRegionBlocks; ++b) {
-                best[b] = invFar;
-                bid[b] = kBackground * 16;
-            }
-            if (!(dskip & 2u)) {
-#pragma unroll
-                for (int sub = 0; sub < SUBS; ++sub) {
-                    if (SUBS > 1 && act[sub] == 0)
-                        continue;
-                    if (nearFree)
-                        rasterRegion<false, 4>(lds.planes, act[sub], recBase + sub * kWave, px, py, tileNear, best, bid);
-                    else
-                        rasterRegion<true, 4>(lds.planes, act[sub], recBase + sub * kWave, px, py, tileNear, best, bid);
-                }
-            }
-            if (full)
-                storeRegion<IDS, true, TEX, OUT, NRM>(p, lds, doRgb, doDepth, rgbTile, depthTile, idsTile, pixOff, fx0, fy,
-                                                      anyTex, px, py, best, bid, nrmLds, nrmTile);
-            else
-                storeRegion<IDS, false, TEX, OUT, NRM>(p, lds, doRgb, doDepth, rgbTile, depthTile, idsTile, pixOff, fx0, fy,
-                                                       anyTex, px, py, best, bid, nrmLds, nrmTile);
-        }
-    }
-    MRX_STAMP(5);
+    constexpr bool POOL = SLOTS == 16 && !TEX && !PV && !COL && !NRM && !LAB;
+#define MRX_PHASE()                                                            \
+    do {                                                                       \
+        if constexpr (POOL)                                                    \
+            asm volatile("" : "+v"(lane), "+s"(pp));                           \
+    } while (0)
+    typedef const __attribute__((address_space(4))) RasterParams KernelParams;
+    typedef std::conditional_t<POOL, KernelParams *, const RasterParams *const> PhaseParams;
+    PhaseParams pp = [&] {
+        if constexpr (POOL)
+            return reinterpret_cast<KernelParams *>(
+                (const __attribute__((address_space(4))) char *)__builtin_amdgcn_kernarg_segment_ptr() + (FAST ? sizeof(GroupHeader) : 0));
+        else
+            return &p;
+    }();
+    if constexpr (!POOL) {
+        constexpr bool FIRST = true, HDR = FAST;
+#include "raster_group_phases.inc"
+    } else {
+        const auto renderGroup = [&](auto firstGroup) __attribute__((always_inline)) {
+            constexpr bool FIRST = decltype(firstGroup)::value, HDR = FAST && FIRST;
+#include "raster_group_phases.inc"
+        };
+        renderGroup(std::true_type {});
+        while (pp->viewPool) {
+            __syncthreads();
+            const uint32_t ticket = __builtin_amdgcn_readfirstlane(lds.poolNext);
+            if (ticket >= pp->numViews - pp->poolFirstView)
+                break;
+            firstView = pp->poolFirstView + ticket;
+            groupViews = groupTiles = 1;
+            firstStrip = 0;
+            numStrips = 8;
+            groupRecs = numPairs = SLOTS;
+            renderGroup(std::false_type {});
+        }
+    }
     MRX_STAMP(6);
     if (stamps && lane == 0)
         stamps[7] = ((unsigned long long)__builtin_amdgcn_s_getreg((31 << 11) | 20) << 32) |
                     (unsigned long long)__builtin_amdgcn_s_getreg((31 << 11) | 4);
 #undef MRX_STAMP
+#undef MRX_PHASE
 }
 
 constexpr int groupThreads(bool tex) { return kWave * groupWaves(tex); }
@@ -1203,8 +920,10 @@
 }
 
 hipError_t launchRaster(const RasterParams &p, uint32_t maxWorldTris,
-                        int32_t variant, hipStream_t stream, int32_t *entry)
-{
+                        int32_t variant, hipStream_t stream, int32_t *entry, ViewPoolSplit *pool)
+{
+    if (pool)
+        *pool = ViewPoolSplit {};
     const uint32_t items = p.numViews * p.tilesFast * p.tilesSlow;
     if (items == 0)
         return hipSuccess;
@@ -1279,14 +998,30 @@
             ct = std::min<uint32_t>((uint32_t)p.grpTilesWanted, tpv);
         }
         gpv = (tpv + ct - 1) / ct;
+        const KernelForm form = groupForm(p);
+        const bool poolShape = form == KernelForm::Uniform && slots == 16 && tpv == 1 && gpv == 1 && !p.anyTextured && p.viewPool &&
+                               p.grpViewsWanted <= 0 && p.grpTilesWanted <= 0 && p.debugSlots == 0;
+        const ViewPoolSplit vp = viewPoolSplit(poolShape, p.numViews, vg, kFill,
+                                               (uint32_t)groupWavesPerSimd(form, 16, false) / 2u * (kFill / 4u),
+                                               p.viewPoolMode, p.viewPoolShare);
+        if (pool)
+            *pool = vp;
+        if (vp.on)
+            vg = vp.staticViews;
+        q.viewPool = vp.on ? p.viewPool : nullptr;
+        q.poolFirstView = vp.firstView;
         q.grpViews = vg;
         q.grpChunkTiles = ct;
         q.grpPerView = gpv;
-        const uint32_t numGroups = gpv == 1 ? (p.numViews + vg - 1) / vg : p.numViews * gpv;
+        const uint32_t numGroups = vp.on ? vp.groups : gpv == 1 ? (p.numViews + vg - 1) / vg : p.numViews * gpv;
         const bool skewable = slots == 16 && tpv == 1 && (vg == 4 || vg == 2);
         q.xcdSkew = (skewable && numGroups >= kFill) ? (vg == 4 ? 3u : 1u) : 0u;
         if (p.xcdSkewWanted >= 0)
             q.xcdSkew = skewable ? (uint32_t)(p.xcdSkewWanted < 8 ? p.xcdSkewWanted : 7) : 0u;
+        if (vp.on) {
+            q.xcdSkew = 0;
+            q.xccReport = nullptr;
+        }
         q.xcdRotate = (tpv == 1 && numGroups >= kFill) ? 1u : 0u;
         if (p.xcdRotateWanted >= 0)
             q.xcdRotate = p.xcdRotateWanted ? 1u : 0u;
@@ -1312,10 +1047,9 @@
             h.first01 = p.uniFirstTri[0] | (p.uniFirstTri[1] << 16);
             h.first23 = p.uniFirstTri[2] | (p.uniFirstTri[3] << 16);
         }
-        const KernelForm form = groupForm(p);
         const bool tex = p.anyTextured != 0;
         const OutSel out = outSelOf(p.rgb, p.depth);
-        const int xmode = slots != 16 ? 0 : ((q.xcdSkew && (p.xcdPhase & 1u)) ? 1 : 0) | (p.xccReport ? 2 : 0);
+        const int xmode = slots != 16 ? 0 : ((q.xcdSkew && (p.xcdPhase & 1u)) ? 1 : 0) | (q.xccReport ? 2 : 0);
         const auto byTexIds = [&](auto f) {
             withBool(tex, [&](auto TEX) { withBool(ids, [&](auto IDS) { f(IDS, TEX); }); });
         };
diff --git a/madrona_renderer_amd/csrc/raster.hpp b/madrona_renderer_amd/csrc/raster.hpp
--- a/madrona_renderer_amd/csrc/raster.hpp
+++ b/madrona_renderer_amd/csrc/raster.hpp
@@ -131,6 +131,9 @@
     uint32_t numMaterials;
     uint32_t *normal;
     const int32_t *instLabel;
+    uint32_t *viewPool;
+    uint32_t poolFirstView;
+    int32_t viewPoolMode, viewPoolShare;
 };
 
 constexpr int32_t kLabelObject = INT32_MIN;
@@ -266,11 +269,40 @@
            (uint64_t)numViews * tpv >= 192ull * cus;
 }
 
+struct ViewPoolSplit {
+    uint32_t on;
+    uint32_t groups;
+    uint32_t staticViews;
+    uint32_t firstView;
+    uint32_t size;
+};
+inline ViewPoolSplit viewPoolSplit(bool shapeOk, uint32_t numViews, uint32_t groupViews, uint32_t fill, uint32_t resident,
+                                   int32_t mode, int32_t share8)
+{
+    ViewPoolSplit s {};
+    if (!shapeOk || mode <= 0 || numViews == 0)
+        return s;
+    if (mode >= 2)
+        groupViews = 4;
+    const uint32_t groups = (numViews + groupViews - 1) / groupViews;
+    if (groupViews != 4 || (mode < 2 && (groups < fill || groups > resident)))
+        return s;
+    uint32_t pooled = share8 > 0 ? ((uint32_t)share8 * groupViews + 4u) / 8u : 0u;
+    pooled = pooled < 1u ? 1u : pooled > groupViews - 1u ? groupViews - 1u : pooled;
+    s.on = 1;
+    s.groups = groups;
+    s.staticViews = groupViews - pooled;
+    const uint64_t owned = (uint64_t)groups * s.staticViews;
+    s.firstView = owned < numViews ? (uint32_t)owned : numViews;
+    s.size = numViews - s.firstView;
+    return s;
+}
+
 enum RasterEntry : int32_t {
     kEntryNone = 0, kEntryGroupFast = 1, kEntryGroup = 2, kEntryChunked = 3, kEntryBrute = 4, kEntryBvh = 5,
 };
 hipError_t launchRaster(const RasterParams &p, uint32_t maxWorldTris,
-                        int32_t variant, hipStream_t stream, int32_t *entry = nullptr);
+                        int32_t variant, hipStream_t stream, int32_t *entry = nullptr, ViewPoolSplit *pool = nullptr);
 
 hipError_t launchBvh(const RasterParams &p, hipStream_t stream);
 constexpr uint32_t kBvhMaxWorldTris = 0x1FFFFEu;
diff --git a/madrona_renderer_amd/csrc/raster_dev.hpp b/madrona_renderer_amd/csrc/raster_dev.hpp
--- a/madrona_renderer_amd/csrc/raster_dev.hpp
+++ b/madrona_renderer_amd/csrc/raster_dev.hpp
@@ -381,11 +381,19 @@
 template <size_t BYTES = sizeof(RasterParams)>
 __device__ __forceinline__ void touchKernelArguments()
 {
-    static_assert(BYTES > 0x180 && BYTES <= 0x240, "seven to nine lines: adjust the offsets below");
+    static_assert(BYTES > 0x180 && BYTES <= 0x280, "seven to ten lines: adjust the offsets below");
     const __attribute__((address_space(4))) char *ka =
         (const __attribute__((address_space(4))) char *)__builtin_amdgcn_kernarg_segment_ptr();
-    uint32_t t0, t1, t2, t3, t4, t5, t6, t7, t8;
-    if (BYTES > 0x200)
+    uint32_t t0, t1, t2, t3, t4, t5, t6, t7, t8, t9;
+    if (BYTES > 0x240)
+        asm volatile("s_load_dword %0, %10, 0x0\n\ts_load_dword %1, %10, 0x40\n\ts_load_dword %2, %10, 0x80\n\t"
+                     "s_load_dword %3, %10, 0xc0\n\ts_load_dword %4, %10, 0x100\n\ts_load_dword %5, %10, 0x140\n\t"
+                     "s_load_dword %6, %10, 0x180\n\ts_load_dword %7, %10, 0x1c0\n\ts_load_dword %8, %10, 0x200\n\t"
+                     "s_load_dword %9, %10, 0x240\n\ts_waitcnt lgkmcnt(0)"
+                     : "=&s"(t0), "=&s"(t1), "=&s"(t2), "=&s"(t3), "=&s"(t4), "=&s"(t5), "=&s"(t6), "=&s"(t7), "=&s"(t8),
+                       "=&s"(t9)
+                     : "s"(ka));
+    else if (BYTES > 0x200)
         asm volatile("s_load_dword %0, %9, 0x0\n\ts_load_dword %1, %9, 0x40\n\ts_load_dword %2, %9, 0x80\n\t"
                      "s_load_dword %3, %9, 0xc0\n\ts_load_dword %4, %9, 0x100\n\ts_load_dword %5, %9, 0x140\n\t"
                      "s_load_dword %6, %9, 0x180\n\ts_load_dword %7, %9, 0x1c0\n\ts_load_dword %8, %9, 0x200\n\t"
diff --git a/madrona_renderer_amd/csrc/raster_group_phases.inc b/madrona_renderer_amd/csrc/raster_group_phases.inc
--- /dev/null
+++ b/madrona_renderer_amd/csrc/raster_group_phases.inc
@@ -0,0 +1,347 @@
+        MRX_PHASE();
+        const uint32_t gNumViews = FIRST ? aNumViews : pp->numViews;
+        const uint32_t gUniInstances = FIRST ? aUniInstances : pp->uniInstances;
+        const uint32_t gUniCams = FIRST ? aUniCams : pp->uniCamsPerWorld;
+        const float *gCamRot = FIRST ? aCamRot : pp->camRot;
+        const float *gCamPos = FIRST ? aCamPos : pp->camPos;
+        const int32_t *gInstObj = FIRST ? aInstObj : pp->instObj;
+        const uint32_t *gInstColor = FIRST ? aInstColor : pp->instColor;
+        const int32_t *gInstMat = FIRST ? aInstMat : pp->instMat;
+        if (!readyItems)
+            for (int i = POOL ? wave * kWave + lane : (int)threadIdx.x; i < numPairs; i += groupWaves(TEX) * kWave)
+                lds.masks[i] = 0u;
+
+        if (wave == groupWaves(TEX) - 1 && lane < (int)groupTiles) {
+            uint32_t vi = (uint32_t)lane, tile = firstTile;
+            if (tilesPerView != 1) {
+                vi = groupViews == 1 ? 0u : (uint32_t)lane / tilesPerView;
+                tile = firstTile + (uint32_t)lane - vi * tilesPerView;
+            }
+            const uint32_t ty = tilesPerView != 1 ? tile / pp->tilesFast : 0u;
+            lds.tileInfo[lane][0] = firstView + vi;
+            lds.tileInfo[lane][1] = (tile - ty * pp->tilesFast) * 64u;
+            lds.tileInfo[lane][2] = ty * 64u;
+            lds.tileInfo[lane][3] = (firstView + vi < gNumViews ? kTileValid : 0u) | ((vi * SLOTS) << 8);
+            if (PV)
+                lds.tileNear[lane] = firstView + vi < gNumViews ? viewProjOf(*(const RasterParams *)pp, true, firstView + vi).invNear : 0.0f;
+        }
+        if (wave == groupWaves(TEX) - 1) {
+            uint32_t base = 0;
+            for (uint32_t c0 = 0; c0 < groupTiles * 8u; c0 += kWave) {
+                const uint32_t c = c0 + (uint32_t)lane;
+                uint32_t strip = c / groupTiles, tile = c - strip * groupTiles;
+                if (tilesPerView != 1) {
+                    tile = c >> 3;
+                    strip = c & 7u;
+                }
+                const uint32_t g = tile * 8u + strip;
+                const bool ok = strip < 8u && g >= firstStrip && g < firstStrip + numStrips;
+                const uint64_t m = __ballot(ok);
+                const uint32_t pos = base + __builtin_popcountll(m & ((1ull << lane) - 1ull));
+                if (readyItems) {
+                    if (strip < 8u)
+                        lds.itemPos[g] = ok ? (uint8_t)pos : (uint8_t)0xFF;
+                } else if (ok) {
+                    lds.itemOrder[pos] = (uint8_t)g;
+                }
+                base += (uint32_t)__builtin_popcountll(m);
+            }
+        }
+        if (wave * kWave < groupRecs) {
+            const int rec = wave * kWave + lane;
+            const int vi = rec / SLOTS, k = rec % SLOTS;
+            const bool recOk = rec < groupRecs;
+            const bool viewOk = recOk && firstView + vi < gNumViews;
+            const uint32_t view = viewOk ? firstView + vi : 0u;
+            WorldTri wt;
+            uint32_t numTris;
+            if (gUniInstances) {
+                const uint32_t kk = (uint32_t)k;
+                const uint32_t pre1 = HDR ? (hPrefix & 255u) : pp->uniPrefix[1], pre2 = HDR ? ((hPrefix >> 8) & 255u) : pp->uniPrefix[2];
+                const uint32_t pre3 = HDR ? ((hPrefix >> 16) & 255u) : pp->uniPrefix[3], pre4 = HDR ? (hPrefix >> 24) : pp->uniPrefix[4];
+                const uint32_t ft0 = HDR ? (hFirst01 & 0xFFFFu) : pp->uniFirstTri[0], ft1 = HDR ? (hFirst01 >> 16) : pp->uniFirstTri[1];
+                const uint32_t ft2 = HDR ? (hFirst23 & 0xFFFFu) : pp->uniFirstTri[2], ft3 = HDR ? (hFirst23 >> 16) : pp->uniFirstTri[3];
+                const uint32_t li = (kk >= pre1 ? 1u : 0u) + (kk >= pre2 ? 1u : 0u) + (kk >= pre3 ? 1u : 0u);
+                const uint32_t pre = li == 0 ? 0u : li == 1 ? pre1 : li == 2 ? pre2 : pre3;
+                const uint32_t first = li == 0 ? ft0 : li == 1 ? ft1 : li == 2 ? ft2 : ft3;
+                uint32_t world = view;
+                if (gUniCams != 1)
+                    world = view / gUniCams;
+                wt.inst = world * gUniInstances + li;
+                wt.tri = first + (kk - pre);
+                numTris = viewOk ? pre4 : 0u;
+                if (kk >= pre4) {
+                    wt.inst = 0;
+                    wt.tri = 0;
+                }
+            } else {
+                wt = pp->viewTris[view * pp->viewTriStride + ((uint32_t)k < pp->viewTriStride ? (uint32_t)k : 0u)];
+                numTris = viewOk ? pp->viewTriCount[view] : 0u;
+            }
+            ViewConst vc;
+            const ViewLight lt = viewLightOf(*(const RasterParams *)pp, PV && LT, view);
+            {
+                const float4 q = *reinterpret_cast<const float4 *>(gCamRot + 4 * view);
+                quatToMat(q.x, q.y, q.z, q.w, vc.Rc);
+#pragma unroll
+                for (int r = 0; r < 3; ++r) {
+                    vc.c[r] = gCamPos[3 * view + r];
+                    vc.lv[r] = dot3(vc.Rc[0][r], vc.Rc[1][r], vc.Rc[2][r],
+                                    lt.toLight[0], lt.toLight[1], lt.toLight[2]);
+                }
+            }
+            TriPlanes c;
+            c.A0 = c.B0 = c.C0 = c.A1 = c.B1 = c.C1 = 0.0f;
+            c.A2 = c.B2 = c.C2 = c.Dx = c.Dy = c.Dc = 0.0f;
+            c.bbX0 = c.bbX1 = c.bbY0 = c.bbY1 = 0.0f;
+            bool valid = false;
+            MRX_STAMP(1);
+            if (recOk) {
+                lds.shade[rec][1] = __int_as_float(-1);
+                if ((uint32_t)k < numTris && !(dskip & 8u)) {
+                    const ViewProj pr = viewProjOf(*(const RasterParams *)pp, PV, view);
+                    const GroupSetupArgs sa = {
+                        HDR ? reinterpret_cast<const ObjTri *>(hGeom) : pp->tris,
+                        HDR ? reinterpret_cast<const TriMat *>(hGeom + geomMatsOffset(hPool)) : pp->triMats,
+                        HDR ? reinterpret_cast<const float *>(hPose + lay.instPos) : pp->instPos,
+                        HDR ? reinterpret_cast<const float *>(hPose + lay.instRot) : pp->instRot,
+                        HDR ? reinterpret_cast<const float *>(hPose + lay.instScale) : pp->instScale,
+                        pr.sx, pr.ox, pr.sz, pr.oz, pr.s6bPad, lt.ambient, lt.diffuse, pp->transposed };
+                    InstXform x;
+                    instanceTransform(sa, vc, wt.inst, x);
+                    if (BYPTR) {
+                        const MatOverride mo = { gInstMat ? gInstMat[wt.inst] : -1, pp->numMaterials, pp->matTable };
+                        if constexpr (NRM)
+                            valid = setupTriangleCore<true, true, true, true>(sa, vc.lv, x, wt.tri, gInstObj[wt.inst], k, c,
+                                                                              lds.shade[rec], lds.cold[rec],
+                                                                              gInstColor ? gInstColor[wt.inst] : 0u, mo,
+                                                                              NormalOut { nrmLds + rec });
+                        else
+                            valid = setupTriangleCore<true, true, true, true>(sa, vc.lv, x, wt.tri, gInstObj[wt.inst], k, c,
+                                                                              lds.shade[rec], lds.cold[rec],
+                                                                              gInstColor ? gInstColor[wt.inst] : 0u, mo);
+                        if (LAB)
+                            applyLabel(lds.shade[rec], pp->instLabel, wt.inst);
+                    } else {
+                    const MatOverride mo = { MAT ? gInstMat[wt.inst] : -1, pp->numMaterials, pp->matTable };
+                    valid = setupTriangleCore<true, OUT != kOutDepth, COL, MAT>(sa, vc.lv, x, wt.tri, gInstObj[wt.inst], k, c,
+                                                                                lds.shade[rec], lds.cold[rec],
+                                                                                COL ? gInstColor[wt.inst] : 0u, mo);
+                    }
+                }
+                MRX_STAMP(2);
+                float4 *dst = reinterpret_cast<float4 *>(lds.planes[rec]);
+                dst[0] = make_float4(c.A0, c.A1, c.A2, c.Dx);
+                dst[1] = make_float4(c.B0, c.B1, c.B2, c.Dy);
+                dst[2] = make_float4(c.C0, c.C1, c.C2, c.Dc);
+                dst[3] = make_float4(c.bbX0, c.bbX1, c.bbY0, c.bbY1);
+                lds.live[rec] = (valid && !(dskip & 4u)) ? 1u : 0u;
+            }
+            if (rec == 0) {
+                lds.nextItem = 0;
+                if (FIRST) {
+                    lds.shade[kBackground][0] = __uint_as_float(0xFF000000u);
+                    lds.shade[kBackground][1] = __int_as_float(-1);
+                    lds.shade[kBackground][2] = __int_as_float(-1);
+                    lds.shade[kBackground][3] = __int_as_float(-1);
+                    if (NRM)
+                        nrmLds[kBackground] = kNormalBackground;
+                }
+            }
+        }
+        __syncthreads();
+        MRX_STAMP(3);
+        MRX_PHASE();
+        const bool drawer = POOL && pp->viewPool && wave == 0 && lane == 0;
+        uint32_t drawn = 0;
+        if (drawer)
+            drawn = atomicAdd(&pp->viewPool[0], 1u);
+
+        constexpr int kPairStride = (groupWaves(TEX) / 4) * kWave;
+        for (int pair = (wave >> 2) * kWave + lane; pair - lane < numPairs; pair += kPairStride) {
+            if (readyItems) {
+                uint32_t m = 0;
+                bool nearOk = false, tex = false;
+                if (pair < numPairs)
+                    m = classifyPair(lds, pair / SLOTS, pair % SLOTS, wave, PV ? lds.tileNear[pair / SLOTS] : invNear, invFar,
+                                     nearOk, tex);
+                m >>= 4 * (wave & 3);
+                const uint64_t l0 = __ballot(m & 1u), r0 = __ballot(m & 2u), l1 = __ballot(m & 4u), r1 = __ballot(m & 8u);
+                const uint64_t near0 = __ballot((m & 3u) && !nearOk), near1 = __ballot((m & 12u) && !nearOk);
+                const uint64_t tex0 = __ballot((m & 3u) && tex), tex1 = __ballot((m & 12u) && tex);
+                if (lane % 16 == 0 && pair < numPairs) {
+                    const uint32_t j = (uint32_t)pair / 16u;
+                    const uint32_t valid = firstView + j < gNumViews ? kItemValid : 0u;
+                    const auto put = [&](uint32_t strip, uint64_t l, uint64_t r, uint64_t nearHit, uint64_t texHit) {
+                        const uint32_t pos = lds.itemPos[j * 8u + strip];
+                        if (pos == 0xFFu)
+                            return;
+                        const uint32_t desc = j | strip << 4 | valid |
+                                              (((nearHit >> lane) & 0xFFFFu) == 0 ? kItemNearFree : 0u) |
+                                              (((texHit >> lane) & 0xFFFFu) != 0 ? kItemAnyTex : 0u);
+                        lds.items[pos] = make_uint2((uint32_t)((l >> lane) & 0xFFFFu) | (uint32_t)((r >> lane) & 0xFFFFu) << 16,
+                                                    desc);
+                    };
+                    put(2u * (wave & 3), l0, r0, near0, tex0);
+                    put(2u * (wave & 3) + 1u, l1, r1, near1, tex1);
+                }
+                continue;
+            }
+            if (pair >= numPairs)
+                continue;
+            bool nearOk, tex;
+            uint32_t m = classifyPair(lds, pair / SLOTS, pair % SLOTS, wave, PV ? lds.tileNear[pair / SLOTS] : invNear,
+                                      invFar, nearOk, tex);
+            if (nearOk)
+                m |= 1u << (16 + (wave & 3));
+            if (m)
+                atomicOr(&lds.masks[pair], m);
+        }
+        __syncthreads();
+        MRX_STAMP(4);
+        MRX_PHASE();
+        if (drawer) {
+            lds.poolNext = drawn;
+            if (drawn >= pp->numViews - pp->poolFirstView && atomicAdd(&pp->viewPool[1], 1u) == gridDim.x - 1u) {
+                atomicExch(&pp->viewPool[0], 0u);
+                atomicExch(&pp->viewPool[1], 0u);
+            }
+        }
+
+        const int lx = lane & 7, ly = lane >> 3;
+        const uint32_t laneOff = (uint32_t)ly * pp->nfast + 4u * lx;
+        int cachedTile = -1, recBase = 0;
+        constexpr int SUBS = (SLOTS + kWave - 1) / kWave;
+        constexpr int LANES = SLOTS < kWave ? SLOTS : kWave;
+        uint32_t view = 0, tileX0 = 0, tileY0 = 0, mask[SUBS] = {};
+        float pxTile[2][kRegionBlocks] = {};
+        bool anyTex = false, nearFree = false, full = false;
+        uint32_t *rgbTile = nullptr;
+        float *depthTile = nullptr;
+        int32_t *idsTile = nullptr;
+        uint32_t *nrmTile = nullptr;
+        const bool doRgb = storesRgb<OUT>(pp->rgb), doDepth = storesDepth<OUT>(pp->depth);
+        uint32_t itemMasks = 0;
+        float tileNear = invNear;
+        if (readyItems) {
+            full = (pp->nfast & 3u) == 0 && 64u <= pp->nfast && 64u <= pp->nslow;
+#pragma unroll
+            for (int hf = 0; hf < 2; ++hf)
+#pragma unroll
+                for (int b = 0; b < kRegionBlocks; ++b)
+                    pxTile[hf][b] = (float)(hf * 32 + 4 * lx + b);
+        }
+        for (;;) {
+            uint32_t item = 0;
+            if (lane == 0)
+                item = atomicAdd(&lds.nextItem, 1u);
+            item = __builtin_amdgcn_readfirstlane(item);
+            if (item >= numStrips)
+                break;
+            int j, strip;
+            if (readyItems) {
+                const uint2 d = lds.items[item];
+                itemMasks = __builtin_amdgcn_readfirstlane(d.x);
+                const uint32_t desc = __builtin_amdgcn_readfirstlane(d.y);
+                if (!(desc & kItemValid))
+                    continue;
+                j = (int)(desc & 15u);
+                strip = (int)((desc >> 4) & 7u);
+                nearFree = (desc & kItemNearFree) != 0;
+                anyTex = (desc & kItemAnyTex) != 0;
+                recBase = j * SLOTS;
+                if (PV)
+                    tileNear = __uint_as_float(__builtin_amdgcn_readfirstlane(__float_as_uint(lds.tileNear[j])));
+                const size_t tileBase = (size_t)(firstView + (uint32_t)j) * pp->nslow * pp->nfast;
+                rgbTile = pp->rgb + tileBase;
+                depthTile = pp->depth + tileBase;
+                idsTile = IDS ? pp->ids + tileBase : nullptr;
+                nrmTile = NRM ? pp->normal + tileBase : nullptr;
+            } else {
+                item = __builtin_amdgcn_readfirstlane((uint32_t)lds.itemOrder[item]);
+                j = (int)(item >> 3);
+                strip = (int)(item & 7u);
+                if (j != cachedTile) {
+                    const uint32_t info = __builtin_amdgcn_readfirstlane(lds.tileInfo[j][3]);
+                    if (!(info & kTileValid))
+                        continue;
+                    cachedTile = j;
+                    recBase = (int)(info >> 8);
+                    view = __builtin_amdgcn_readfirstlane(lds.tileInfo[j][0]);
+                    tileX0 = __builtin_amdgcn_readfirstlane(lds.tileInfo[j][1]);
+                    tileY0 = __builtin_amdgcn_readfirstlane(lds.tileInfo[j][2]);
+                    if (PV)
+                        tileNear = __uint_as_float(__builtin_amdgcn_readfirstlane(__float_as_uint(lds.tileNear[j])));
+                    const size_t tileBase = ((size_t)view * pp->nslow + tileY0) * pp->nfast + tileX0;
+                    rgbTile = pp->rgb + tileBase;
+                    depthTile = pp->depth + tileBase;
+                    idsTile = IDS ? pp->ids + tileBase : nullptr;
+                    nrmTile = NRM ? pp->normal + tileBase : nullptr;
+                    full = (pp->nfast & 3u) == 0 && tileX0 + 64u <= pp->nfast && tileY0 + 64u <= pp->nslow;
+                    anyTex = false;
+                    nearFree = true;
+#pragma unroll
+                    for (int sub = 0; sub < SUBS; ++sub) {
+                        const int slot = sub * kWave + lane;
+                        mask[sub] = lane < LANES ? lds.masks[j * SLOTS + slot] : 0u;
+                        const int32_t tex = lane < LANES ? __float_as_int(lds.shade[recBase + slot][1]) : -1;
+                        anyTex = anyTex || __ballot((mask[sub] & 0xFFFFu) != 0 && tex >= 0) != 0;
+                        nearFree = nearFree &&
+                                   __ballot((mask[sub] & 0xFFFFu) != 0 && ((mask[sub] >> 16) & 0xFu) != 0xFu) == 0;
+                    }
+#pragma unroll
+                    for (int hf = 0; hf < 2; ++hf)
+#pragma unroll
+                        for (int b = 0; b < kRegionBlocks; ++b)
+                            pxTile[hf][b] = (float)(tileX0 + hf * 32 + 4 * lx + b);
+                }
+            }
+            const uint32_t fy = tileY0 + strip * 8 + ly;
+            const float py = (float)fy;
+#pragma unroll
+            for (int hf = 0; hf < 2; ++hf) {
+                const uint32_t fx0 = tileX0 + hf * 32 + 4 * lx;
+                const uint32_t pixOff = (uint32_t)(strip * 8) * pp->nfast + hf * 32 + laneOff;
+                uint64_t act[SUBS];
+                bool any = false;
+#pragma unroll
+                for (int sub = 0; sub < SUBS; ++sub) {
+                    act[sub] = readyItems ? (uint64_t)((itemMasks >> (16 * hf)) & 0xFFFFu)
+                                         : __ballot((mask[sub] >> (2 * strip + hf)) & 1u);
+                    any = any || act[sub] != 0;
+                }
+                if (!any) {
+                    if (full)
+                        storeBackground<IDS, true, NRM>(*(const RasterParams *)pp, doRgb, doDepth, rgbTile, depthTile, idsTile, pixOff, fx0, fy, nrmTile);
+                    else
+                        storeBackground<IDS, false, NRM>(*(const RasterParams *)pp, doRgb, doDepth, rgbTile, depthTile, idsTile, pixOff, fx0, fy, nrmTile);
+                    continue;
+                }
+                const float (&px)[kRegionBlocks] = pxTile[hf];
+                float best[kRegionBlocks];
+                int32_t bid[kRegionBlocks];
+#pragma unroll
+                for (int b = 0; b < kRegionBlocks; ++b) {
+                    best[b] = invFar;
+                    bid[b] = kBackground * 16;
+                }
+                if (!(dskip & 2u)) {
+#pragma unroll
+                    for (int sub = 0; sub < SUBS; ++sub) {
+                        if (SUBS > 1 && act[sub] == 0)
+                            continue;
+                        if (nearFree)
+                            rasterRegion<false, 4>(lds.planes, act[sub], recBase + sub * kWave, px, py, tileNear, best, bid);
+                        else
+                            rasterRegion<true, 4>(lds.planes, act[sub], recBase + sub * kWave, px, py, tileNear, best, bid);
+                    }
+                }
+                if (full)
+                    storeRegion<IDS, true, TEX, OUT, NRM>(*(const RasterParams *)pp, lds, doRgb, doDepth, rgbTile, depthTile, idsTile, pixOff, fx0, fy,
+                                                          anyTex, px, py, best, bid, nrmLds, nrmTile);
+                else
+                    storeRegion<IDS, false, TEX, OUT, NRM>(*(const RasterParams *)pp, lds, doRgb, doDepth, rgbTile, depthTile, idsTile, pixOff, fx0, fy,
+                                                           anyTex, px, py, best, bid, nrmLds, nrmTile);
+            }
+        }
+        MRX_STAMP(5);
```
